# Pixel-Talk/CanonSwap

Measured on AMD Instinct MI355X. Metric: frames/sec at 512x512 (generator hot path F->W->T->R->W->G), higher is better.
Workload: dtype f16; 1 GPU; BASELINE configs[2]: 512x512 video, 64 frames batched per launch on each GPU, steady state over 1280 frames (20 launches per GPU) (256x256 crops in, random-init weights of the real architecture); frames_per_launch_per_gpu=64, frames_total=1280, parallelism=frame-shard x1, identities_resident=1, latency_mode=False, accumulate=fp32, debug_decodes=False

## Files before the change

canonswap_amd/_lib.py:

```python
from __future__ import annotations

import ctypes as C
import os
import subprocess

HERE = os.path.dirname(os.path.abspath(__file__))
CSRC = os.path.join(HERE, "csrc")
SOURCES = [os.path.join(CSRC, f) for f in ("conv_halo.hip", "conv_wide.hip", "conv_lat.hip", "vol32.hip", "vol32_fused.hip", "kernels.hip", "motion.hip", "imgops.hip", "engine.hip")]
TEST_SRC = os.path.join(os.path.dirname(HERE), "tests", "csrc", "test_igemm.hip")
TEST_LIB_PATH = os.path.join(os.path.dirname(HERE), "tests", "libcanonswap_test.so")
HEADERS = [os.path.join(CSRC, f) for f in ("common.h", "conv_epilogue.h", "conv_halo_kernel.h")] + \
          [os.path.join(os.path.dirname(HERE), "include", "canonswap_hip.h")]
HALO_NGROUPS = 8
OBJ_DIR = os.path.join(HERE, "build")
LIB_PATH = os.environ.get("CANONSWAP_LIB") or os.path.join(HERE, "libcanonswap_hip.so")
ABI_SYMBOLS = [
    "cs_create", "cs_destroy", "cs_last_error", "cs_abi_version", "cs_upload", "cs_finalize_weights", "cs_set_identity", "cs_set_latency_mode",
    "cs_extract_feature_3d", "cs_warp", "cs_warp_out", "cs_swap", "cs_swap_ids", "cs_swap_frames_ids", "cs_refine", "cs_warp_forward", "cs_spade_decode",
    "cs_pack_u8", "cs_unpack_u8", "cs_soft_erosion", "cs_prepare_crops", "cs_warp_affine_u8", "cs_warp_affine_f32", "cs_paste_back",
    "cs_motion_extract", "cs_motion_keypoints", "cs_soft_erosion_frames", "cs_paste_back_batch", "cs_swap_frames", "cs_animate_frames", 
    "cs_resize_half_bilinear", "cs_motion_keypoints_driven", "cs_paste_back_shared", "cs_crop_frames", "cs_face_masks", "cs_profile_begin", "cs_profile_end", "cs_profile_exec_flops", "cs_op_conv", "cs_op_grid_sample3d",
    "cs_op_chan_stats", "cs_op_chan_stats_partial_floats", "cs_op_pair_ragged", "cs_op_resblock3d", "cs_op_t_mask",
    "cs_op_t_style", "cs_op_t_modulate", "cs_op_t_read", "cs_op_t_layer",
    "cs_op_m_stem", "cs_op_m_dwln", "cs_op_m_ln_s2d", "cs_op_m_grn", "cs_op_m_head", "cs_op_m_pointwise",
# ... 105 lines not shown
            waits = waits[:4]
            loads = [(i, re.search(r"global_load_dwordx4 v\[(\d+):(\d+)\], v\[\d+:\d+\], off", l)) for i, l in enumerate(body)]
            loads = [(i, int(q.group(1))) for i, q in loads if q]
            prime = [r for i, r in loads if i < waits[0]][-4 * wch:]
            if len(prime) != 4 * wch:
                raise RuntimeError(f"isa_check: {name}: the prologue primes {len(prime)} ring registers, expected {4 * wch}")
            for k, w in enumerate(waits):
                slot = prime[k * wch:(k + 1) * wch]
                end = waits[k + 1] if k + 1 < 4 else len(body)
                seg = body[w:end]
                rel = [i for i, r in loads if w < i < end and r in slot]
                if len(rel) < wch:
                    raise RuntimeError(f"isa_check: {name}: ring slot {k} is not reloaded into v{slot} after its wait")
                first_reload = min(rel) - w
                uses = [j for j, l in enumerate(seg[:first_reload]) if "v_mfma" in l and any(f"v[{r}:{r + 3}]" in l for r in slot)]
                if not uses:
                    raise RuntimeError(f"isa_check: {name}: no MFMA reads ring slot {k} (v{slot}) between its wait and its reload")
            tail = "\n".join(body[waits[-1]:])
            if "s_waitcnt vmcnt(0)" not in tail:
                raise RuntimeError(f"isa_check: {name}: the ring is not drained (s_waitcnt vmcnt(0)) before the epilogue")
            seen[name] = len(waits)
    if not seen:
        raise RuntimeError("isa_check: no dynamic-shape conv_halo kernel found in the objects (name mangling changed?)")
    return seen


def _isa_check_lat(obj_dir: str, objdump: str) -> dict:
    import re
    oname = "conv_lat.o"
    obj = os.path.join(obj_dir, oname)
    subprocess.run([objdump, "--offloading", obj], check=True, capture_output=True)
    co = obj + ".0.hipv4-amdgcn-amd-amdhsa--gfx950"
    try:
        txt = subprocess.run([objdump, "-d", "--no-show-raw-insn", co], check=True, capture_output=True, text=True).stdout
    finally:
        for f in os.listdir(obj_dir):
            if f.startswith(oname + ".0."):
                os.remove(os.path.join(obj_dir, f))
    seen = {}
    for m in re.finditer(r"^[0-9a-f]+ <(\S*conv_lat_kernel\S*)>:\n(.*?)(?=^[0-9a-f]+ <|\Z)", txt, re.S | re.M):
        name, body = m.group(1), [l.split("//")[0].strip() for l in m.group(2).split("\n")]
        body = [l for l in body if l]
        mf = [i for i, l in enumerate(body) if l.startswith("v_mfma")]
        if not mf:
            raise RuntimeError(f"isa_check: {name}: no MFMA")
        if any(l.startswith(("s_cbranch", "s_branch")) for l in body[mf[0]:mf[-1]]):
            raise RuntimeError(f"isa_check: {name}: a branch inside the K loop (the walk assumes straight-line code)")
        for i, l in enumerate(body):
            if re.search(r"\bm0\b", l):
                ok = l.startswith("s_mov_b32 m0,") and any(b.startswith("buffer_load") and b.endswith("lds") for b in body[i + 1:i + 3])
                if not ok:
                    raise RuntimeError(f"isa_check: {name}: `{l}` touches m0 outside the hidden LDS-DMA sequence")
        nvm, open_dma, nbar, ndma = 0, [], 0, 0
        for i, l in enumerate(body[:mf[-1] + 1]):
            op = l.split()[0]
            if op.startswith(("global_load", "buffer_load", "global_store", "buffer_store", "scratch_load", "scratch_store")):
                if op.startswith("buffer_load") and l.endswith("lds"):
                    open_dma.append(nvm); ndma += 1
                nvm += 1
            if op == "s_barrier":
                nbar += 1
                w = next((body[j] for j in range(i - 1, max(i - 6, -1), -1) if body[j].startswith("s_waitcnt") and "vmcnt" in body[j]), None)
                if w is None and not open_dma:
                    continue
                if w is None:
                    raise RuntimeError(f"isa_check: {name}: barrier {nbar} of the K loop has no vmcnt wait in front of it")
                n = int(re.search(r"vmcnt\((\d+)\)", w).group(1))
                for idx in open_dma:
                    if nvm - idx - 1 < n:
                        raise RuntimeError(f"isa_check: {name}: `{w}` before barrier {nbar} does not cover a DMA piece issued {nvm - idx - 1} vector-memory instructions earlier")
                open_dma = []
        if open_dma:
            raise RuntimeError(f"isa_check: {name}: {len(open_dma)} DMA pieces are never waited for at a chunk head")
        if len(mf) not in (8 * 6 * 8, 8 * 6 * 16) or ndma != 24:
            raise RuntimeError(f"isa_check: {name}: {len(mf)} MFMAs / {ndma} DMA instructions, expected 384 or 768 / 24")
        seen[name] = len(mf)
    if not seen:
        raise RuntimeError("isa_check: no conv_lat kernel found in conv_lat.o (name mangling changed?)")
    return seen


def _isa_check_wide(obj_dir: str, objdump: str) -> dict:
    seen = _isa_check_ring(obj_dir, objdump, "conv_wide.o", r"\S*conv_wide_kernel\S*", 18 * 64)
    seen.update(_isa_check_ring(obj_dir, objdump, "conv_halo_g1.o", r"_Z16conv_halo_kernelILi32ELi8ELi5ELi2ELi2ELi0ELb1ELb0ELi[789]E\S*", None))
    return seen


def _isa_check_ring(obj_dir: str, objdump: str, oname: str, name_re: str, expect_mfma) -> dict:
    import re
    obj = os.path.join(obj_dir, oname)
    subprocess.run([objdump, "--offloading", obj], check=True, capture_output=True)
    co = obj + ".0.hipv4-amdgcn-amd-amdhsa--gfx950"
    try:
        txt = subprocess.run([objdump, "-d", "--no-show-raw-insn", co], check=True, capture_output=True, text=True).stdout
    finally:
        for f in os.listdir(obj_dir):
            if f.startswith(oname + ".0."):
                os.remove(os.path.join(obj_dir, f))
    seen = {}
    for m in re.finditer(r"^[0-9a-f]+ <(" + name_re + r")>:\n(.*?)(?=^[0-9a-f]+ <|\Z)", txt, re.S | re.M):
        name, body = m.group(1), m.group(2).split("\n")
        writer, waited, issued, nmfma = {}, {}, {}, 0
        pending, nvm = [], 0
        mf = [i for i, l in enumerate(body) if "v_mfma" in l]
        lo, hi = (mf[0], mf[-1]) if mf else (0, 0)
        for li, l in enumerate(body):
            t = l.split("//")[0].strip()
            if not t:
                continue
            op = t.split()[0]
            if op.startswith("s_waitcnt") and "vmcnt" in t:
                n = int(re.search(r"vmcnt\((\d+)\)", t).group(1))
                for r in waited:
                    if nvm - issued.get(r, -1) - 1 >= n:
                        waited[r] = True
                pending = [q for q in pending if nvm - q[1] - 1 < n]
            if op.startswith(("s_cbranch", "s_branch", "s_endpgm")) or li < lo:
                pending = []
            if pending and not op.startswith(("s_", "global_store", "buffer_store", "ds_write", "scratch_store")):
                mm0 = re.match(r"\S+\s+(v\[(\d+):(\d+)\]|v(\d+))", t)
                if mm0 and not (op.startswith("buffer_load") and t.endswith("lds")):
                    dst = set(range(int(mm0.group(2)), int(mm0.group(3)) + 1)) if mm0.group(2) else {int(mm0.group(4))}
                    for regs, _ in pending:
                        if regs & dst:
                            raise RuntimeError(f"isa_check: {name}: `{t}` writes v{sorted(regs & dst)} while an untracked ring load into them is in flight")
            if op.startswith(("global_load", "buffer_load", "global_store", "buffer_store", "scratch_load", "scratch_store", "global_atomic")):
                if op.startswith("global_load_dwordx4") and li >= lo:
                    q = re.match(r"\S+\s+v\[(\d+):(\d+)\]", t)
                    if q:
                        pending.append((set(range(int(q.group(1)), int(q.group(2)) + 1)), nvm))
                nvm += 1
            if op.startswith("v_mfma"):
                ops = re.findall(r"([av])\[(\d+):(\d+)\]", t)
                if len(ops) < 4 or ops[1][0] != "v":
                    raise RuntimeError(f"isa_check: {name}: MFMA with a weight operand outside the VGPRs: {t}")
                nmfma += 1
                for r in range(int(ops[1][1]), int(ops[1][2]) + 1):
                    if not writer.get(r, "").startswith("global_load_dwordx4"):
                        raise RuntimeError(f"isa_check: {name}: v{r}, a weight operand of `{t}`, was last written by `{writer.get(r)}` (a copy of a ring register?)")
                    if not waited.get(r, False):
                        raise RuntimeError(f"isa_check: {name}: no vmcnt wait between the ring load of v{r} and `{t}`")
                continue
            if op.startswith(("global_store", "buffer_store", "ds_write", "scratch_store", "s_", "buffer_load_dwordx4")) and "lds" in t + " lds" and not op.startswith("global_load"):
                if not op.startswith(("v_", "ds_read", "global_load", "scratch_load")):
                    continue
            mm = re.match(r"\S+\s+(v\[(\d+):(\d+)\]|v(\d+))", t)
            if mm and not op.startswith(("global_store", "buffer_store", "ds_write", "scratch_store")) and not (op.startswith("buffer_load") and t.endswith("lds")):
                rng = range(int(mm.group(2)), int(mm.group(3)) + 1) if mm.group(2) else [int(mm.group(4))]
                is_vm = op.startswith(("global_load", "buffer_load", "scratch_load"))
                for r in rng:
                    writer[r] = op
                    waited[r] = False
                    issued[r] = (nvm - 1) if is_vm else -1
        if expect_mfma is not None and nmfma != expect_mfma:
            raise RuntimeError(f"isa_check: {name}: {nmfma} MFMAs in the kernel, expected {expect_mfma}")
        seen[name] = nmfma
    if not seen:
        raise RuntimeError(f"isa_check: no kernel matching {name_re} found in {oname} (name mangling changed?)")
    return seen


class ConvDesc(C.Structure):
    _fields_ = [
        ("in_", C.c_void_p), ("in_sN", C.c_long), ("in_sD", C.c_long), ("in_sH", C.c_long), ("in_sW", C.c_long),
        ("N", C.c_int), ("D", C.c_int), ("H", C.c_int), ("W", C.c_int), ("Cin", C.c_int), ("up_shift", C.c_int),
        ("KD", C.c_int), ("KH", C.c_int), ("KW", C.c_int),
        ("wgt", C.c_void_p), ("Cout_pad", C.c_int), ("Cout", C.c_int),
# ... 106 lines not shown
```

canonswap_amd/csrc/common.h:

```cpp
#pragma once
#include <hip/hip_runtime.h>
#include <stdint.h>

typedef _Float16 half_t;
typedef _Float16 h8_t __attribute__((ext_vector_type(8)));
typedef _Float16 h4_t __attribute__((ext_vector_type(4)));
typedef float f4_t __attribute__((ext_vector_type(4)));

enum { ACT_NONE = 0, ACT_RELU = 1, ACT_LRELU = 2, ACT_SIGMOID = 3, ACT_GELU = 4 };
enum { MODE_STD = 0, MODE_TBLEND = 1, MODE_SPADE = 2, MODE_PIXSHUF = 3,
       MODE_STDSTAT = 4 };
enum { CFG_128x128 = 0, CFG_128x64 = 1, CFG_256x32 = 2, CFG_256x16 = 3 };
enum { CFG_H_128x128 = 10, CFG_H_128x64 = 11, CFG_H_256x32 = 12, CFG_H_128x32 = 13, CFG_H_128x16 = 14, CFG_H_256x16 = 15,
       CFG_H_SK128x32 = 16 , CFG_H_128x256 = 17,
       CFG_H_128x160 = 18 ,
       CFG_H_256x160 = 19 ,
       CFG_H_256x64 = 20 ,
       CFG_VOL32 = 30 , CFG_WIDE = 31 ,
       CFG_LAT = 32  };

struct TDesc {
    void* p;
    long sN, sD, sH, sW;
};

struct ConvParams {
    const half_t* in;
    const half_t* zero;
    long in_sN, in_sD, in_sH, in_sW;
    int N, D, H, W;
    int inD;
    int Cin;
    int cg, cg_cin;
    long in_sG;
    int nchunks;
    int up_shift;
    int KD, KH, KW, PD, PH, PW;
    const half_t* wgt;
    const long* wofs;
    const int* wslot;
    int Cout_pad;
    int Cout;
    int lgTW, lgTH, lgTD;
    int nTW, nTH, nTD, nTN;
    const float* bias;
    const float* bias2;
    int act0;
    float slope0;
    TDesc res;
    int res_f32;
    int res_shift;
    const float* pixscale;
    int ps_stride;
    TDesc out0;
    int out0_f32;
    const float* s2;
    const float* t2;
    int act1;
    float slope1;
    TDesc out1;
    const float* stats;
    float* stat_out;
    float* sk_out;
    int sk_splits;
    int ragged;
    unsigned mg_ncb, mg_tw, mg_th, mg_td;
    int hilo;
    int xcd_map;
    float* kw_out;
    int ep_general;
    int pool_hw;
    int spmul;
    const half_t* xs_w; TDesc xs_res, xs_out; int xs_cout;
    int persist_total;
    unsigned in_sample_bytes;
    int nphase;
    long ph_wofs[4];
    unsigned ph_ooff[4];
    int ph_PH[4], ph_PW[4];
    int xf_kind;
    int v32_srows;
    TDesc xf_y, xf_res, xf_out;
    const float* xf_stats; const float* xf_gamma; const float* xf_beta;
    float xf_slope;
#ifdef CS_TIMELINE
    unsigned long long* tl;
    long tl_cap;
#endif
};

__device__ __forceinline__ float gn_scale(float rstd, float gamma) { return rstd * gamma; }
__device__ __forceinline__ float gn_shift(float mean, float sc, float beta) { return fmaf(-mean, sc, beta); }
__device__ __forceinline__ float gn_lrelu(float v, float sc, float sh, float rr, float slope)
{
    float a = fmaf(v, sc, sh);
    a = a + rr;
    return fmaxf(a, a * slope);
}

#define CS_CHECK_HIP(expr)                                                                  \
// ... 87 lines not shown
```

canonswap_amd/csrc/conv_epilogue.h:

```cpp
#pragma once
#include "common.h"

#ifndef EP_TL
#define EP_TL(i) do { } while (0)
#endif
typedef unsigned int ep_u4_t __attribute__((ext_vector_type(4)));
typedef unsigned int ep_u2_t __attribute__((ext_vector_type(2)));

static inline int ep_check_extents(const ConvParams& p, const char* who)
{
    auto span = [&](const TDesc& t) -> long {
        return (long)(p.N - 1) * t.sN + (long)(p.D - 1) * t.sD + (long)(p.H - 1) * t.sH + (long)(p.W - 1) * t.sW + p.Cout;
    };
    auto wide = [&](const TDesc& t) { return t.sD >= (1L << 23) || t.sH >= (1L << 23) || t.sW >= (1L << 23); };
    const long lim = 1L << 31;
    long ph_max = 0;
    for (int z = 0; z < p.nphase && z < 4; ++z) ph_max = p.ph_ooff[z] > ph_max ? (long)p.ph_ooff[z] : ph_max;
    if ((p.out0.p && span(p.out0) + ph_max >= lim) || (p.out1.p && span(p.out1) >= lim) || (p.res.p && span(p.res) >= lim)) {
        cs_set_error("%s: a tensor of this launch spans 2^31 elements or more (32-bit in-tensor offsets)", who);
        return -1;
    }
    if ((p.out0.p && wide(p.out0)) || (p.out1.p && wide(p.out1)) || (p.res.p && wide(p.res)) || p.D >= (1 << 22) || p.H >= (1 << 22) ||
        p.W >= (1 << 22)) {
        cs_set_error("%s: an axis stride of 2^23 elements or more (24-bit multiplies in the addressing)", who);
// ... 97 lines not shown
#else
#define EP_STORE_COND
#endif
#define CONV_EPILOGUE_EARLY_FETCH() \
    ep_u2_t ep_xpre[EP_EARLY ? EP_WPX0 : 1][EP_EARLY ? (WCH + 1) / 2 : 1]; \
    if constexpr (EP_EARLY) { \
        int xlw, xlh, xld, xln; \
        { int t = l15p; xlw = t & mW; t >>= lgTW; xlh = t & mH; t >>= lgTH; xld = t & mD; t >>= lgTD; xln = t; } \
        const int xrs = p.res_shift, xnb = tn * (BM >> lgS); \
        const unsigned xlane = (unsigned)((xnb + xln) * (int)p.res.sN + __mul24((td << lgTD) + xld, (int)p.res.sD) + \
                                          __mul24(((th << lgTH) + xlh) >> xrs, (int)p.res.sH) + __mul24(((tw << lgTW) + xlw) >> xrs, (int)p.res.sW)); \
_Pragma("unroll") \
        for (int pi = 0; pi < EP_WPX0; ++pi) { \
            int bw, bh, bd, bn; \
            { int t = (ep_wpx0 * EP_WPX0 + pi) << 4; bw = t & mW; t >>= lgTW; bh = t & mH; t >>= lgTH; bd = t & mD; t >>= lgTD; bn = t; } \
            const unsigned xb = xlane + (unsigned)(bn * (int)p.res.sN + bd * (int)p.res.sD + (bh >> xrs) * (int)p.res.sH + (bw >> xrs) * (int)p.res.sW); \
_Pragma("unroll") \
            for (int ci = 0; ci < WCH; ci += 2) { \
                const int cb = ep_chan(EP_PAIR, 2, n0 + wch * WCH * 16, ci, l4); \
                ep_u2_t q2; q2[0] = 0u; q2[1] = 0u; \
                if (p.res.p && xnb + xln + bn < p.N && cb < p.Cout) q2 = *(const ep_u2_t*)((const half_t*)p.res.p + (xb + (unsigned)cb)); \
                ep_xpre[pi][ci / 2] = q2; \
            } \
        } \
    }

template <int N> __device__ __forceinline__ float ep_row_shl(float a)
{
#ifdef EP_HOST_EMULATION
    (void)a;
    return 0.f;
#else
    return __builtin_bit_cast(float, __builtin_amdgcn_update_dpp(0, __builtin_bit_cast(int, a), 0x100 | N, 0xf, 0xf, true));
#endif
}

__device__ __forceinline__ float ep_row_sum16(float a)
{
#ifdef EP_HOST_EMULATION
    for (int o = 1; o < 16; o <<= 1) a += __shfl_xor(a, o, 64);
    return a;
#else
    a += __builtin_bit_cast(float, __builtin_amdgcn_update_dpp(0, __builtin_bit_cast(int, a), 0x101, 0xf, 0xf, true));
    a += __builtin_bit_cast(float, __builtin_amdgcn_update_dpp(0, __builtin_bit_cast(int, a), 0x102, 0xf, 0xf, true));
    a += __builtin_bit_cast(float, __builtin_amdgcn_update_dpp(0, __builtin_bit_cast(int, a), 0x104, 0xf, 0xf, true));
    a += __builtin_bit_cast(float, __builtin_amdgcn_update_dpp(0, __builtin_bit_cast(int, a), 0x108, 0xf, 0xf, true));
    return a;
#endif
}

#define EP_STAT_FLUSH(sg) \
    if (EP_STAT) { \
        const int ep_tiles = p.nTW * p.nTH * p.nTD; \
        const int ep_nblk = EP_NBLK_V; \
        const int ep_blk = EP_BLK_V(sg); \
_Pragma("unroll") \
        for (int ci = 0; ci < WCH; ci += CSTEP) { \
            const int cb = ep_chan(EP_PAIR, CSTEP, n0 + wch * WCH * 16, ci, l4); \
            float ep_pa[4], ep_pb[4]; \
_Pragma("unroll") \
            for (int r = 0; r < 4; ++r) { \
                ep_pa[r] = ep_row_sum16(ep_sum[EP_STAT ? ci : 0][r]); ep_pb[r] = ep_row_sum16(ep_sq[EP_STAT ? ci : 0][r]); \
                ep_sum[EP_STAT ? ci : 0][r] = 0.f; ep_sq[EP_STAT ? ci : 0][r] = 0.f; \
            } \
             \
            if (l15 == 0 && cb < p.Cout) { \
                float4* dst = (float4*)(p.stat_out + (((long)tn * ep_nblk + ep_blk) * p.Cout + cb) * 2); \
                dst[0] = make_float4(ep_pa[0], ep_pb[0], ep_pa[1], ep_pb[1]); \
                dst[1] = make_float4(ep_pa[2], ep_pb[2], ep_pa[3], ep_pb[3]); \
            } \
        } \
    }

#ifndef EP_GSEL_V
#define EP_GSEL_V 0
#endif
#ifndef EP_BLK_V
#define EP_BLK_V(sg) ((tile_lin % ep_tiles) * (BM / (EP_SG * 16)) + ep_wpx * (EP_WPX / EP_SG) + (sg))
#define EP_NBLK_V (ep_tiles * (BM / (EP_SG * 16)))
#endif
#ifndef EP_SLICE_FENCE
#define EP_SLICE_FENCE
#endif
#ifndef EP_FG
#define EP_FG 8
#endif
#ifndef EP_FG_F32
#define EP_FG_F32 4
#endif
#ifndef EP_FG_STAT
#define EP_FG_STAT 4
#endif
#ifndef EP_PIPE_V
#define EP_PIPE_V 0
#endif
#ifndef EP_O0_EXTRA_V
#define EP_O0_EXTRA_V 0u
#endif
#ifndef EP_POOL_WSH_V
#define EP_POOL_WSH_V 0
#define EP_POOL_HSH_V 0
#endif
#define EP_POOLB 128
#ifndef EP_SPMUL_V
#define EP_SPMUL_V 0
#endif
#ifndef EP_O1ONLY_V
#define EP_O1ONLY_V 0
#endif
#ifndef EP_MLIN_V
#define EP_MLIN_V 0
#endif
#ifndef EP_DUP_V
#define EP_DUP_V 0
#endif
#define EP_SPMULB 256
#define EP_GELUB 512
#define EP_FETCH_ROUND(PG0, BI) \
    if (EP_PF && !EP_EARLY && (ep_fetch || ep_has_ps)) { \
_Pragma("unroll") \
        for (int g = 0; g < EP_G; ++g) { \
            int bw, bh, bd, bn; \
            { int t = (ep_wpx * EP_WPX + (PG0) + g) << 4; bw = t & mW; t >>= lgTW; bh = t & mH; t >>= lgTH; bd = t & mD; t >>= lgTD; bn = t; } \
            if (!EPFAST && ep_nb + ep_ln + bn >= p.N) continue; \
            if (ep_has_ps) ep_ps2[BI][g] = p.pixscale[ep_lane_ps + (unsigned)((((bn * p.D + bd) * p.H + bh) * p.W + bw) * p.ps_stride)]; \
            if (ep_fetch) { \
                const unsigned xb = ep_lane_res + (unsigned)(bn * (int)p.res.sN + bd * (int)p.res.sD + (bh >> ep_rs) * (int)p.res.sH + \
                                                            (bw >> ep_rs) * (int)p.res.sW); \
_Pragma("unroll") \
                for (int ci = 0; ci < WCH; ci += CSTEP) { \
                    const int cb = ep_chan(EP_PAIR, CSTEP, n0 + wch * WCH * 16, ci, l4); \
                    if (!EPALL && cb >= p.Cout) continue; \
                    if (ep_res32) ep_raw2[BI][g][(EP_PF ? ci / CSTEP : 0)] = *(const ep_u4_t*)((const float*)p.res.p + (xb + (unsigned)cb)); \
                    else if (ep_mr && ep_second(EP_PAIR, ci)) {  } \
                    else if (ep_mr && (EPALL || cb + 4 < p.Cout)) ep_raw2[BI][g][(EP_PF ? ci / CSTEP : 0)] = *(const ep_u4_t*)((const half_t*)p.res.p + (xb + (unsigned)cb)); \
                    else { \
                        const ep_u2_t q2 = *(const ep_u2_t*)((const half_t*)p.res.p + (xb + (unsigned)cb)); \
                        ep_raw2[BI][g][(EP_PF ? ci / CSTEP : 0)][0] = q2[0]; ep_raw2[BI][g][(EP_PF ? ci / CSTEP : 0)][1] = q2[1]; \
                    } \
                } \
            } \
        } \
    }
#define CONV_EPILOGUE_IMPL(EPCODE) \
    constexpr int EPF = (EPCODE); \
    constexpr bool EPFAST = EPF >= 0; \
    constexpr bool EPALL = EPFAST && ((EPF >> 6) & 1) == 0;       \
    constexpr bool EP_POOL = EPFAST && ((EPF >> 7) & 1) != 0 && (EP_POOL_WSH_V) > 0;       \
    constexpr int EP_PS = EP_POOL ? 1 : 0; \
    constexpr bool EP_GELU = EPFAST && ((EPF >> 9) & 1) != 0;           \
    const bool ep_spm = EPFAST ? (((EPF >> 8) & 1) != 0) : ((MODE == MODE_STD) && p.spmul != 0); \
    constexpr bool EP_POOL_HB = EP_POOL && (EP_POOL_HSH_V) == 0;       \
    float ep_phold[EP_POOL_HB ? WCH : 1][4];                            \
    const bool ep_has_res = EPFAST ? ((EPF & 3) != 0) : (p.res.p != nullptr); \
    const bool ep_res32 = EPFAST ? ((EPF & 3) == 2) : (p.res_f32 != 0); \
    const bool ep_has_o0 = EPFAST ? (((EPF >> 2) & 1) != 0) : (p.out0.p != nullptr); \
    const bool ep_o032 = EPFAST ? (((EPF >> 3) & 1) != 0) : (p.out0_f32 != 0); \
    const bool ep_has_o1 = EPFAST ? (((EPF >> 4) & 1) != 0) : (p.out1.p != nullptr); \
    const bool ep_has_ps = EPFAST ? (((EPF >> 5) & 1) != 0) : (p.pixscale != nullptr); \
    constexpr int CSTEP = (MODE == MODE_TBLEND || MODE == MODE_SPADE) ? 2 : 1; \
     \
    float4 ep_bias[WCH], ep_bias2[WCH], ep_s2[WCH], ep_t2[WCH], ep_mean[WCH], ep_rstd[WCH]; \
_Pragma("unroll") \
    for (int ci = 0; ci < WCH; ci += CSTEP) { \
        const int cb = ep_chan(EP_PAIR, CSTEP, n0 + wch * WCH * 16, ci, l4); \
        const bool cok = EPALL || cb < p.Cout; \
        ep_bias[ci] = (cok && p.bias) ? *(const float4*)(p.bias + cb) : make_float4(0.f, 0.f, 0.f, 0.f); \
        ep_bias2[ci] = (cok && MODE == MODE_SPADE) ? *(const float4*)(p.bias2 + cb) : make_float4(0.f, 0.f, 0.f, 0.f); \
        ep_s2[ci] = (cok && p.s2) ? *(const float4*)(p.s2 + cb) : make_float4(1.f, 1.f, 1.f, 1.f); \
        ep_t2[ci] = (cok && p.s2) ? *(const float4*)(p.t2 + cb) : make_float4(0.f, 0.f, 0.f, 0.f); \
        if ((MODE == MODE_SPADE || ep_spm) && cok) {  \
            const float4 q0 = *(const float4*)(p.stats + ((long)tn * p.Cout + cb) * 2); \
            const float4 q1 = *(const float4*)(p.stats + ((long)tn * p.Cout + cb) * 2 + 4); \
            ep_mean[ci] = make_float4(q0.x, q0.z, q1.x, q1.z); ep_rstd[ci] = make_float4(q0.y, q0.w, q1.y, q1.w); \
        } else { ep_mean[ci] = make_float4(0.f, 0.f, 0.f, 0.f); ep_rstd[ci] = make_float4(1.f, 1.f, 1.f, 1.f); } \
    } \
    const float ep_sl0 = lin_slope(p.act0, p.slope0), ep_sl1 = lin_slope(p.act1, p.slope1); \
    constexpr bool EP_STAT = (MODE == MODE_STDSTAT);  \
    constexpr int EP_SC = EP_STAT ? WCH : 1; \
     \
    constexpr int EP_SG = EP_WPX > 4 ? 4 : EP_WPX; \
    float ep_sum[EP_SC][4], ep_sq[EP_SC][4]; \
_Pragma("unroll") \
    for (int ci = 0; ci < EP_SC; ++ci) \
_Pragma("unroll") \
        for (int r = 0; r < 4; ++r) { ep_sum[ci][r] = 0.f; ep_sq[ci][r] = 0.f; } \
     \
    constexpr bool EP_PF = (WCH != 5); \
     \
    constexpr int EP_G = (EP_GSEL_V) > 0 ? (EP_GSEL_V) : !EP_PF ? 1 : (EP_WPX < 8 ? EP_WPX : (MODE == MODE_TBLEND ? 8 : (WCH == 4 ? (EPFAST ? (EP_STAT ? EP_FG_STAT : ((EPF & 3) == 2 ? EP_FG_F32 : EP_FG)) : (EP_STAT ? 1 : 2)) : 4))); \
    constexpr int EP_NCI = EP_PF ? (WCH + CSTEP - 1) / CSTEP : 1; \
    const bool ep_fetch = EP_PF && ep_has_res; \
     \
    const bool ep_m0 = EP_PAIR != 0 && !ep_o032 && (EPFAST || ep_al8(p.out0)); \
    const bool ep_m1 = EP_PAIR != 0 && (EPFAST || ep_al8(p.out1)); \
    const bool ep_mr = EP_PAIR != 0 && EP_PF && !ep_res32 && (EPFAST || ep_al8(p.res)); \
    const int ep_rshift = (MODE == MODE_SPADE || ep_spm) ? p.res_shift : 0; \
     \
    int ep_lw, ep_lh, ep_ld, ep_ln; \
    { int t = l15p; ep_lw = t & mW; t >>= lgTW; ep_lh = t & mH; t >>= lgTH; ep_ld = t & mD; t >>= lgTD; ep_ln = t; } \
    const int ep_w0 = tw << lgTW, ep_h0 = th << lgTH, ep_d0 = td << lgTD, ep_nb = tn * (BM >> lgS); \
    const int ep_rs = (MODE == MODE_SPADE || ep_spm) ? p.res_shift : 0; \
     \
    const bool ep_tn1 = (BM >> lgS) == 1; \
    const unsigned ep_lane_res = (unsigned)(ep_nb * (int)p.res.sN + (ep_tn1 ? 0 : ep_ln * (int)p.res.sN) + __mul24(ep_d0 + ep_ld, (int)p.res.sD) + \
                                            __mul24((ep_h0 + ep_lh) >> ep_rs, (int)p.res.sH) + __mul24((ep_w0 + ep_lw) >> ep_rs, (int)p.res.sW)); \
    const unsigned ep_lane_o0 = (EP_O0_EXTRA_V) + (unsigned)(ep_nb * (int)p.out0.sN + (ep_tn1 ? 0 : ep_ln * (int)p.out0.sN) + __mul24(ep_d0 + ep_ld, (int)p.out0.sD) + \
                                           __mul24((ep_h0 + ep_lh) >> EP_PS, (int)p.out0.sH) + __mul24((ep_w0 + ep_lw) >> EP_PS, (int)p.out0.sW)); \
     \
    const bool ep_pool_lane = !EP_POOL || (lane & ((EP_POOL_WSH_V) | (EP_POOL_HSH_V))) == 0; \
    const unsigned ep_lane_o1 = (EP_O0_EXTRA_V) + (unsigned)(ep_nb * (int)p.out1.sN + (ep_tn1 ? 0 : ep_ln * (int)p.out1.sN) + __mul24(ep_d0 + ep_ld, (int)p.out1.sD) + \
                                           __mul24(ep_h0 + ep_lh, (int)p.out1.sH) + __mul24(ep_w0 + ep_lw, (int)p.out1.sW)); \
    const unsigned ep_lane_ps = (unsigned)(((((ep_nb + ep_ln) * p.D + ep_d0 + ep_ld) * p.H + ep_h0 + ep_lh) * p.W + ep_w0 + ep_lw) * p.ps_stride); \
     \
    const unsigned ep_lane_px = (unsigned)((((ep_nb + ep_ln) * 3) * 2 * p.H + 2 * (ep_h0 + ep_lh)) * 2 * p.W + 2 * (ep_w0 + ep_lw)); \
     \
    constexpr bool EP_PIPE = (EP_PIPE_V) != 0 && EP_G < EP_WPX; \
    ep_u4_t ep_raw2[EP_PIPE ? 2 : 1][EP_G][EP_NCI]; float ep_ps2[EP_PIPE ? 2 : 1][EP_G]; \
    if (EP_PIPE) { EP_FETCH_ROUND(0, 0) } \
_Pragma("unroll") \
    for (int pg = 0; pg < EP_WPX; pg += EP_G) { \
    const int ep_bi = EP_PIPE ? ((pg / EP_G) & 1) : 0; \
    if (!EP_PIPE) { EP_FETCH_ROUND(pg, 0) } \
    else if (pg + EP_G < EP_WPX) { EP_FETCH_ROUND(pg + EP_G, EP_PIPE ? (((pg / EP_G) + 1) & 1) : 0) } \
    ep_u4_t (&ep_raw)[EP_G][EP_NCI] = ep_raw2[ep_bi]; float (&ep_ps)[EP_G] = ep_ps2[ep_bi]; \
    if (pg == 0) EP_TL(6); \
_Pragma("unroll") \
    for (int g = 0; g < EP_G; ++g) { \
        const int pi = pg + g; \
        if (pi == 1) EP_TL(7); \
        if (pi > 0 && pi % EP_SG == 0) { EP_STAT_FLUSH(pi / EP_SG - 1) } \
        int bw, bh, bd, bn; \
        { int t = (ep_wpx * EP_WPX + pi) << 4; bw = t & mW; t >>= lgTW; bh = t & mH; t >>= lgTH; bd = t & mD; t >>= lgTD; bn = t; } \
        if (!EPFAST && ep_nb + ep_ln + bn >= p.N) continue; \
        float ps = 1.f; \
        if (ep_has_ps) ps = EP_PF ? ep_ps[g] : p.pixscale[ep_lane_ps + (unsigned)((((bn * p.D + bd) * p.H + bh) * p.W + bw) * p.ps_stride)]; \
        const unsigned xb = ep_lane_res + (unsigned)(bn * (int)p.res.sN + bd * (int)p.res.sD + (bh >> ep_rs) * (int)p.res.sH + (bw >> ep_rs) * (int)p.res.sW); \
        const unsigned ob0 = ep_lane_o0 + (unsigned)(bn * (int)p.out0.sN + bd * (int)p.out0.sD + (bh >> EP_PS) * (int)p.out0.sH + (bw >> EP_PS) * (int)p.out0.sW); \
        const unsigned ob1 = ep_lane_o1 + (unsigned)(bn * (int)p.out1.sN + bd * (int)p.out1.sD + bh * (int)p.out1.sH + bw * (int)p.out1.sW); \
        float ep_vh[4] = {0.f, 0.f, 0.f, 0.f}, ep_uh[4] = {0.f, 0.f, 0.f, 0.f};       \
_Pragma("unroll") \
        for (int ci = 0; ci < WCH; ci += CSTEP) { \
            const int cb = ep_chan(EP_PAIR, CSTEP, n0 + wch * WCH * 16, ci, l4); \
            if (!EPALL && cb >= p.Cout) continue; \
            float rr[4] = {0.f, 0.f, 0.f, 0.f};      \
            if (ep_has_res) { \
                if (EP_EARLY) { \
                    const h4_t hx = __builtin_bit_cast(h4_t, ep_xpre[EP_EARLY ? pi : 0][EP_EARLY ? ci / 2 : 0]); \
_Pragma("unroll") \
                    for (int r = 0; r < 4; ++r) rr[r] = (float)hx[r]; \
                } else if (EP_PF) { \
                    const bool ep_hi = ep_mr && ep_second(EP_PAIR, ci);       \
                    const ep_u4_t q4 = ep_raw[g][(EP_PF ? ci / CSTEP : 0)]; \
                    const ep_u4_t qp = ep_raw[g][(EP_PF && ep_second(EP_PAIR, ci) ? ci / CSTEP - 1 : 0)]; \
                    if (ep_res32) { \
                        const f4_t qf = __builtin_bit_cast(f4_t, q4);      \
_Pragma("unroll") \
                        for (int r = 0; r < 4; ++r) rr[r] = qf[r]; \
                    } else { \
                        ep_u2_t q2; q2[0] = ep_hi ? qp[2] : q4[0]; q2[1] = ep_hi ? qp[3] : q4[1]; \
                        const h4_t hx = __builtin_bit_cast(h4_t, q2); \
_Pragma("unroll") \
                        for (int r = 0; r < 4; ++r) rr[r] = (float)hx[r]; \
                    } \
                } else { \
                    load4(p.res, ep_res32, (long)(xb + (unsigned)cb), rr); \
                } \
            } \
            float v[4]; \
            if (MODE == MODE_TBLEND) { \
_Pragma("unroll") \
                for (int r = 0; r < 4; ++r) \
                    v[r] = ps * (ep_acc[ci + CSTEP - 1][pi][r] + ((const float*)&ep_bias[ci])[r]) + (1.f - ps) * ep_acc[ci][pi][r]; \
            } else if (MODE == MODE_SPADE) { \
_Pragma("unroll") \
                for (int r = 0; r < 4; ++r) { \
                    const float gm = ep_acc[ci][pi][r] + ((const float*)&ep_bias[ci])[r]; \
                    const float bt = ep_acc[ci + CSTEP - 1][pi][r] + ((const float*)&ep_bias2[ci])[r]; \
                    v[r] = fmaf((rr[r] - ((const float*)&ep_mean[ci])[r]) * ((const float*)&ep_rstd[ci])[r], 1.f + gm, bt); \
                } \
            } else { \
_Pragma("unroll") \
                for (int r = 0; r < 4; ++r) v[r] = ep_acc[ci][pi][r] + ((const float*)&ep_bias[ci])[r]; \
                if (ep_spm) { \
_Pragma("unroll") \
                    for (int r = 0; r < 4; ++r) v[r] = ((rr[r] - ((const float*)&ep_mean[ci])[r]) * ((const float*)&ep_rstd[ci])[r]) * (1.f + v[r]); \
                } \
            } \
_Pragma("unroll") \
             \
            for (int r = 0; r < 4; ++r) v[r] = EP_GELU ? gelu_act(v[r]) : ((EP_HEAVY && !EPFAST) ? apply_act(v[r], p.act0, p.slope0) : lin_act(v[r], ep_sl0)); \
            if (MODE == MODE_PIXSHUF) { \
                const int c = cb >> 2; \
                if (c < 3) { \
                    float* o = (float*)p.out0.p; \
                    const unsigned W2 = 2u * (unsigned)p.W, H2 = 2u * (unsigned)p.H; \
                    const unsigned base = ep_lane_px + ((unsigned)(bn * 3 + c) * H2 + 2u * (unsigned)bh) * W2 + 2u * (unsigned)bw; \
                    *(float2*)(o + base) = make_float2(v[0], v[1]); \
                    *(float2*)(o + base + W2) = make_float2(v[2], v[3]); \
                } \
                continue; \
            } \
             \
            if (MODE != MODE_SPADE && !ep_spm) { \
_Pragma("unroll") \
                for (int r = 0; r < 4; ++r) v[r] += rr[r]; \
            } \
            if (MODE == MODE_STD || MODE == MODE_STDSTAT) { \
_Pragma("unroll") \
                for (int r = 0; r < 4; ++r) v[r] *= ps; \
            } \
            if (EP_POOL_HB) {  \
_Pragma("unroll") \
                for (int r = 0; r < 4; ++r) { \
                    if ((pi & 1) == 0) ep_phold[EP_POOL_HB ? ci : 0][r] = v[r]; \
                    else { \
// ... 105 lines not shown
```

canonswap_amd/csrc/conv_halo.hip:

```cpp
#include "conv_halo_kernel.h"

#ifndef HALO_GROUP
#define HALO_GROUP (-1)
#endif
#define IN_GROUP(g) (HALO_GROUP == -1 || HALO_GROUP == (g))
#define NOT_MINE (-2)

template <int CK, int WPX, int WCH, int WVP, int WVC, int MODE, bool SK, int STV>
static int launch_halo_cfg(const ConvParams& p, hipStream_t st)
{
    if constexpr (STV != 0) {
        using SS = StaticShape<STV>;
        if (p.KD == SS::KD && p.KH == SS::KH && p.KW == SS::KW && p.lgTW == SS::LW && p.lgTH == SS::LH && p.lgTD == SS::LD &&
            p.nchunks % (CK / 32) == 0)
            return launch_halo_st<CK, WPX, WCH, WVP, WVC, MODE, SK, STV>(p, st);
    }
    if constexpr (WCH == 4 && MODE == MODE_STDSTAT) {
        cs_set_error("conv_halo: the 128x256 statistics tile exists for the static shapes only (%dx%dx%d taps, tile 2^%d x 2^%d x 2^%d)",
                     p.KD, p.KH, p.KW, p.lgTW, p.lgTH, p.lgTD);
        return -1;
    } else {
        return launch_halo_st<CK, WPX, WCH, WVP, WVC, MODE, SK, 0>(p, st);
    }
}

#define HALO_CASE(CFG, WPX, WCH, WVP, WVC, MODE, SK, ST2D, ST3D)                                         \
    if (cfg == CFG && mode == MODE) {                                                                    \
        if (ck == 64) return launch_halo_cfg<64, WPX, WCH, WVP, WVC, MODE, SK, ST2D>(p, st);            \
        if (stv == 1) return launch_halo_cfg<32, WPX, WCH, WVP, WVC, MODE, SK, ST2D>(p, st);            \
        if (stv == 5 && ST3D == 2) return launch_halo_cfg<32, WPX, WCH, WVP, WVC, MODE, SK, (ST3D == 2 ? 5 : 0)>(p, st); \
        return launch_halo_cfg<32, WPX, WCH, WVP, WVC, MODE, SK, ST3D>(p, st);                           \
    }

#define GROUP_FN(g) int launch_conv_halo_g##g(const ConvParams& p, int cfg, int ck, int mode, int stv, hipStream_t st)
GROUP_FN(0); GROUP_FN(1); GROUP_FN(2); GROUP_FN(3); GROUP_FN(4); GROUP_FN(5); GROUP_FN(6); GROUP_FN(7);

#if IN_GROUP(0)
GROUP_FN(0)
{
    (void)stv;
    if (p.KD == 3 && p.KH == 2 && p.KW == 2 && ck == 32 && mode == MODE_STD) {
        if (cfg == CFG_H_256x32) return launch_halo_cfg<32, 4, 2, 4, 1, MODE_STD, false, 12>(p, st);
        if (cfg == CFG_H_128x64) return launch_halo_cfg<32, 4, 2, 2, 2, MODE_STD, false, 13>(p, st);
        if (cfg == CFG_H_128x128 && p.lgTW == 2) return launch_halo_cfg<32, 8, 2, 1, 4, MODE_STD, false, 17>(p, st);
        if (cfg == CFG_H_128x128) return launch_halo_cfg<32, 8, 2, 1, 4, MODE_STD, false, 13>(p, st);
    }
    if (mode == MODE_STD && p.KD == 1 && p.KH == 1 && p.KW == 1) {
        if (cfg == CFG_H_128x128 && ck == 32) return launch_halo_cfg<32, 8, 2, 1, 4, MODE_STD, false, 15>(p, st);
        if (cfg == CFG_H_128x64 && ck == 64) return launch_halo_cfg<64, 4, 2, 2, 2, MODE_STD, false, 15>(p, st);
        if (cfg == CFG_H_128x64 && ck == 32) return launch_halo_cfg<32, 4, 2, 2, 2, MODE_STD, false, 15>(p, st);
        if (cfg == CFG_H_128x32 && ck == 64) return launch_halo_cfg<64, 2, 2, 4, 1, MODE_STD, false, 15>(p, st);
        if (cfg == CFG_H_128x32 && ck == 32) return launch_halo_cfg<32, 2, 2, 4, 1, MODE_STD, false, 15>(p, st);
    }
    return NOT_MINE;
}
#endif

#if IN_GROUP(1)
GROUP_FN(1)
{
    if (cfg == CFG_H_128x128 && mode == MODE_STD && ck == 64 && p.KD == 1 && p.KH <= 2 && p.KW <= 2) {
        if (p.KH == 2 && p.KW == 2) return launch_halo_cfg<64, 8, 2, 1, 4, MODE_STD, false, 10>(p, st);
        if (p.KH == 2) return launch_halo_cfg<64, 8, 2, 1, 4, MODE_STD, false, 11>(p, st);
        if (p.KW == 2) return launch_halo_cfg<64, 8, 2, 1, 4, MODE_STD, false, 14>(p, st);
        return launch_halo_cfg<64, 8, 2, 1, 4, MODE_STD, false, 15>(p, st);
    }
    if (cfg == CFG_H_256x64 && mode == MODE_STD && ck == 32) return launch_halo_cfg<32, 8, 2, 2, 2, MODE_STD, false, 7>(p, st);
    if (cfg == CFG_H_256x64 && ck == 64) {
        if (p.KD != 1 || p.KH != 3 || p.KW != 3 || p.lgTW != 4 || p.lgTH != 4 || p.lgTD != 0) {
            cs_set_error("conv_halo: the 2-D 256x64 tile runs 3x3 convs on 16x16 tiles only");
            return -1;
        }
        if (mode == MODE_STD) return launch_halo_st<64, 8, 2, 2, 2, MODE_STD, false, 16>(p, st);
        if (mode == MODE_STDSTAT) return launch_halo_st<64, 8, 2, 2, 2, MODE_STDSTAT, false, 16>(p, st);
    }
    if (cfg == CFG_H_256x160 && mode == MODE_STD && ck == 32) {
        if (p.KD == 7 && p.lgTW == 2) return launch_halo_cfg<32, 8, 5, 2, 2, MODE_STD, false, 9>(p, st);
        if (p.KD == 7) return launch_halo_cfg<32, 8, 5, 2, 2, MODE_STD, false, 8>(p, st);
        return launch_halo_cfg<32, 8, 5, 2, 2, MODE_STD, false, 7>(p, st);
    }
    if (cfg == CFG_H_128x160 && mode == MODE_STD && ck == 32) {
        if (stv == 4) return launch_halo_cfg<32, 4, 5, 2, 2, MODE_STD, false, 4>(p, st);
        if (stv == 6) return launch_halo_cfg<32, 4, 5, 2, 2, MODE_STD, false, 6>(p, st);
        return launch_halo_cfg<32, 4, 5, 2, 2, MODE_STD, false, 2>(p, st);
    }
    return NOT_MINE;
}
#endif

#if IN_GROUP(2)
GROUP_FN(2)
{
    HALO_CASE(CFG_H_128x256, 8, 4, 1, 4, MODE_STD, false, 1, 0)
    HALO_CASE(CFG_H_128x256, 8, 4, 1, 4, MODE_TBLEND, false, 1, 0)
    return NOT_MINE;
}
#endif

#if IN_GROUP(3)
GROUP_FN(3)
{
    HALO_CASE(CFG_H_128x256, 8, 4, 1, 4, MODE_SPADE, false, 1, 0)
    HALO_CASE(CFG_H_128x256, 8, 4, 1, 4, MODE_STDSTAT, false, 1, 0)
    return NOT_MINE;
}
#endif

#if IN_GROUP(4)
GROUP_FN(4)
{
    HALO_CASE(CFG_H_128x128, 8, 2, 1, 4, MODE_STD, false, 1, 2)
    HALO_CASE(CFG_H_128x128, 8, 2, 1, 4, MODE_STDSTAT, false, 1, 0)
    return NOT_MINE;
}
#endif

#if IN_GROUP(5)
GROUP_FN(5)
{
    HALO_CASE(CFG_H_128x128, 8, 2, 1, 4, MODE_TBLEND, false, 1, 0)
    HALO_CASE(CFG_H_128x128, 8, 2, 1, 4, MODE_SPADE, false, 1, 0)
    HALO_CASE(CFG_H_128x64, 4, 2, 2, 2, MODE_STDSTAT, false, 1, 0)
    return NOT_MINE;
}
#endif

#if IN_GROUP(6)
GROUP_FN(6)
{
    HALO_CASE(CFG_H_128x64, 4, 2, 2, 2, MODE_STD, false, 1, 2)
    HALO_CASE(CFG_H_256x32, 4, 2, 4, 1, MODE_STD, false, 0, 3)
    HALO_CASE(CFG_H_256x32, 4, 2, 4, 1, MODE_STDSTAT, false, 0, 3)
    return NOT_MINE;
}
#endif

#if IN_GROUP(7)
GROUP_FN(7)
{
    HALO_CASE(CFG_H_128x32, 2, 2, 4, 1, MODE_STD, false, 0, 2)
    HALO_CASE(CFG_H_128x16, 2, 1, 4, 1, MODE_STD, false, 1, 0)
    HALO_CASE(CFG_H_256x16, 4, 1, 4, 1, MODE_PIXSHUF, false, 0, 0)
    HALO_CASE(CFG_H_SK128x32, 8, 2, 4, 1, MODE_STD, true, 0, 0)
    return NOT_MINE;
}
#endif

#if IN_GROUP(0) && defined(CS_TIMELINE)
unsigned long long* g_cs_tl = nullptr;
long g_cs_tl_cap = 0;
extern "C" void cs_debug_set_timeline(void* buf, long cap) { g_cs_tl = (unsigned long long*)buf; g_cs_tl_cap = cap; }
#endif

#if IN_GROUP(0)
int launch_conv_halo(const ConvParams& p, int cfg, int ck, int mode, hipStream_t st)
{
    if (mode == MODE_STD && p.stat_out) mode = MODE_STDSTAT;
    const int stv = p.KD == 1 ? 1 : (p.KD == 7 ? (p.lgTW == 1 ? 6 : 4) : (p.lgTD == 4 ? 3 : (p.lgTD == 3 ? 5 : 2)));
    int r;
#define TRY_GROUP(g) if ((r = launch_conv_halo_g##g(p, cfg, ck, mode, stv, st)) != NOT_MINE) return r;
    TRY_GROUP(0) TRY_GROUP(1) TRY_GROUP(2) TRY_GROUP(3) TRY_GROUP(4) TRY_GROUP(5) TRY_GROUP(6) TRY_GROUP(7)
#undef TRY_GROUP
// ... 5 lines not shown
```

canonswap_amd/csrc/conv_halo_kernel.h:

```cpp
#pragma once
#include <type_traits>
#include <utility>
#include <cstdlib>
#include "common.h"
#ifdef CS_TIMELINE
#define EP_TL(i) TL_STAMP(i)
#endif
#define EP_POOL_WSH_V EP_POOL_WSH_K
#define EP_POOL_HSH_V EP_POOL_HSH_K
#define EP_SPMUL_V EP_SPMUL_K
#define EP_DUP_V EP_DUP_K
#define EP_MLIN_V EP_MLIN_K
#define EP_O1ONLY_V EP_O1ONLY_K
#define EP_O0_EXTRA_V ep_o0_extra
#include "conv_epilogue.h"

typedef unsigned int u4_t __attribute__((ext_vector_type(4)));
__device__ __forceinline__ unsigned mdiv(unsigned u, unsigned magic) { return magic ? __umulhi(u, magic) : u; }

template <int OFF>
__device__ __forceinline__ void wfrag_load(u4_t& dst, const half_t* ptr)
{
    asm volatile("global_load_dwordx4 %0, %1, off offset:%2" : "=v"(dst) : "v"(ptr), "n"(OFF));
}
template <int N>
__device__ __forceinline__ void wait_vmcnt_le()
{
    asm volatile("s_waitcnt vmcnt(%0)" ::"n"(N) : "memory");
}

#ifdef CS_TIMELINE
extern unsigned long long* g_cs_tl;
extern long g_cs_tl_cap;
#define TL_STAMP(i) do { __builtin_amdgcn_sched_barrier(0); tl_t[i] = __builtin_amdgcn_s_memtime(); __builtin_amdgcn_sched_barrier(0); } while (0)
#else
#define TL_STAMP(i) do { } while (0)
#endif

template <int ST> struct StaticShape { static constexpr int KD = 0, KH = 0, KW = 0, LW = 0, LH = 0, LD = 0; };
template <> struct StaticShape<1> { static constexpr int KD = 1, KH = 3, KW = 3, LW = 4, LH = 3, LD = 0; };
template <> struct StaticShape<2> { static constexpr int KD = 3, KH = 3, KW = 3, LW = 3, LH = 3, LD = 1; };
template <> struct StaticShape<3> { static constexpr int KD = 3, KH = 3, KW = 3, LW = 2, LH = 2, LD = 4; };
template <> struct StaticShape<4> { static constexpr int KD = 7, KH = 7, KW = 1, LW = 3, LH = 3, LD = 1; };
template <> struct StaticShape<5> { static constexpr int KD = 3, KH = 3, KW = 3, LW = 2, LH = 2, LD = 3; };
template <> struct StaticShape<6> { static constexpr int KD = 7, KH = 7, KW = 1, LW = 1, LH = 3, LD = 3; };
template <> struct StaticShape<7> { static constexpr int KD = 3, KH = 3, KW = 3, LW = 3, LH = 3, LD = 2; };
template <> struct StaticShape<8> { static constexpr int KD = 7, KH = 7, KW = 1, LW = 1, LH = 3, LD = 4; };
template <> struct StaticShape<9> { static constexpr int KD = 7, KH = 7, KW = 1, LW = 2, LH = 3, LD = 3; };
template <> struct StaticShape<16> { static constexpr int KD = 1, KH = 3, KW = 3, LW = 4, LH = 4, LD = 0; };
template <> struct StaticShape<12> { static constexpr int KD = 3, KH = 2, KW = 2, LW = 2, LH = 2, LD = 4; };
template <> struct StaticShape<13> { static constexpr int KD = 3, KH = 2, KW = 2, LW = 3, LH = 3, LD = 1; };
template <> struct StaticShape<17> { static constexpr int KD = 3, KH = 2, KW = 2, LW = 2, LH = 2, LD = 3; };
template <> struct StaticShape<10> { static constexpr int KD = 1, KH = 2, KW = 2, LW = 4, LH = 3, LD = 0; };
template <> struct StaticShape<11> { static constexpr int KD = 1, KH = 2, KW = 1, LW = 4, LH = 3, LD = 0; };
template <> struct StaticShape<14> { static constexpr int KD = 1, KH = 1, KW = 2, LW = 4, LH = 3, LD = 0; };
template <> struct StaticShape<15> { static constexpr int KD = 1, KH = 1, KW = 1, LW = 4, LH = 3, LD = 0; };

template <int CK, int WPX, int WCH, int WVP, int ST, int MODE> constexpr int halo_pad()
{
#ifdef CS_LDS_V1
    return 1;
#else
    if (CK == 64 && WCH == 4 && WPX == 8 && ST == 1) return 2;
    if (CK == 32 && WCH == 5 && WPX == 8 && (ST == 7 || ST == 8 || ST == 9)) return 2;
    if (CK == 64 && WCH == 2 && WPX == 8 && WVP == 2 && ST == 16) return 2;
    if (CK == 32 && WCH == 2 && WPX == 8 && ST == 1 && MODE == MODE_SPADE) return 2;
#ifdef CS_LDS_V32
    if (CK == 32 && WCH == 2 && WPX == 4 && WVP == 4 && ST == 3) return 2;
#endif
    return 1;
#endif
}
template <int ST, int PAD> constexpr int halo_hi()
{
    if (PAD == 2) return ST == 3 ? 16 : (ST == 9 ? 19 : ((ST == 7 || ST == 8) ? 15 : (ST == 16 ? 13 : 8)));
    return ST == 4 ? 18 : ((ST == 3 || ST == 7 || ST == 8 || ST == 9) ? 13 : (ST == 12 ? 9 : 8));
}
template <int ST, int PAD> __host__ __device__ constexpr int halo_lane_pos(int l)
{
#ifdef CS_LDS_V1
    return l;
#else
    using SS = StaticShape<ST>;
    if (ST == 0 || SS::KW != 3 || SS::LW > 3 || SS::LW < 2) return l;
    if (SS::LW == 2 && PAD == 2) return ((l & 1) << 1) | ((l & 2) << 2) | ((l >> 2) & 1) | ((l & 8) >> 1);
    return ((l & 1) << 1) | ((l & 2) << 1) | ((l >> 2) & 1) | (l & 8);
#endif
}

template <class F, int... I> __device__ __forceinline__ void halo_static_for_impl(F&& f, std::integer_sequence<int, I...>) { (f(std::integral_constant<int, I>{}), ...); }
template <int N, class F> __device__ __forceinline__ void halo_static_for(F&& f) { halo_static_for_impl(static_cast<F&&>(f), std::make_integer_sequence<int, N>{}); }

template <int WCH, int PFS, int HI, int ST0>
constexpr int halo_ring_young(int st, int L, int NP, bool dma_cur)
{
    auto dma = [&](int u, bool on) { return (on && u >= ST0 && u < ST0 + HI) ? 1 : 0; };
    auto cur_before = [&](int from_step ) {
        int n = 0;
        for (int u = from_step; u < st; ++u) n += (u >= 1 ? WCH : 0) + dma(u, dma_cur);
        return n;
    };
    if (st >= PFS) {
        const int u0 = st - PFS + 1;
        return dma(u0, dma_cur) + cur_before(u0 + 1);
    }
    const int prime = (PFS - 1 - st) * WCH + cur_before(0);
    int g = 0;
    if (NP % PFS == 0) g = st + NP - PFS + 1;
    else { for (int u = NP - PFS + 1; u <= NP; ++u) if ((u - 1) % PFS == st) g = u; }
    int carried = dma(g, true);
    for (int u = g + 1; u <= NP; ++u) carried += WCH + (u < NP ? dma(u, true) : 0);
    carried += cur_before(0);
    return prime < carried ? prime : carried;
}

template <int ST, int PAD> constexpr int halo_pool_shift(int bit)
{
    for (int b = 0; b < 4; ++b) if (halo_lane_pos<ST, PAD>(1 << b) == (1 << bit)) return 1 << b;
    return 0;
}

template <int WCH, int ST> constexpr bool halo_phase_group() { return !(ST == 0 && WCH >= 4); }

template <int CK, int WPX, int WCH, int WVP, int MODE, bool SK, int ST> constexpr bool halo_pool2d()
{
    using SS = StaticShape<ST>;
    return ST != 0 && !SK && MODE == MODE_STD && CK == 32 && WPX == 8 && WVP == 1 && (WCH == 2 || WCH == 4) && SS::KD == 1 && SS::KH == 3 && SS::KW == 3 &&
           SS::LW == 4 && SS::LH == 3 && SS::LD == 0;
}

template <int CK, int WPX, int WCH, int WVP, int WVC, int MODE, bool DB, bool SK, int ST>
__global__ void __launch_bounds__(256, (WCH == 4 ? 2 : ((WCH == 2 && WPX == 8 && !SK && ST != 0) ? (WVP == 2 ? 2 : 3) : 1))) conv_halo_kernel(const ConvParams p)
{
    using SS = StaticShape<ST>;
    static_assert(ST == 0 || !SK, "static shapes are not combined with split-K");
    constexpr int BM = SK ? WPX * 16 : WPX * 16 * WVP;
    constexpr int BN = WCH * 16 * WVC;
    constexpr int SL = CK / 8;
    constexpr int PAD = halo_pad<CK, WPX, WCH, WVP, ST, MODE>();
    constexpr int SLP = SL + PAD;
    constexpr bool EP_POOLK = ST != 0 && !SK && MODE == MODE_STD && WCH == 2 && SS::KD == 3 && SS::KH == 3 && SS::KW == 3 && (SS::LW == 3 || SS::LW == 2) && SS::LH >= 1;
    constexpr bool EP_POOLK2 = halo_pool2d<CK, WPX, WCH, WVP, MODE, SK, ST>();
    constexpr bool XSK = ST == 1 && !SK && MODE == MODE_STD && CK == 64 && WCH == 4 && WPX == 8 && WVP == 1;
#ifdef CS_NO_SPMUL_FAST
    constexpr bool EP_SPMUL_K = false;
#else
    constexpr bool EP_SPMUL_K = ST == 1 && !SK && MODE == MODE_STD && CK == 64 && WCH == 4 && WPX == 8 && WVP == 1;
#endif
    constexpr bool EP_O1ONLY_K = ST == 16 && !SK && MODE == MODE_STD;
    constexpr bool EP_MLIN_K = ST == 15 && !SK && MODE == MODE_STD;
    constexpr bool EP_DUP_K = (ST == 11 || ST == 14 || ST == 15) && !SK && MODE == MODE_STD && WCH == 2 && WPX == 8;
    constexpr int EP_POOL_WSH_K = EP_POOLK ? halo_pool_shift<ST, PAD>(0) : (EP_POOLK2 ? 1 : 0);
    constexpr int EP_POOL_HSH_K = EP_POOLK ? halo_pool_shift<ST, PAD>(SS::LW) : 0;
    constexpr int VS = SLP * 16;
    constexpr int HI = halo_hi<ST, PAD>();
    constexpr int KH32 = CK / 32;
    constexpr int PFD = 4;
    constexpr int SKS = SK ? 4 : 1;
    static_assert(WVP * WVC == 4, "4 waves per workgroup");
    static_assert(!SK || (WVC == 1 && WPX == 8), "split-K variants: every wave covers all 128 positions");

    extern __shared__ __attribute__((aligned(16))) unsigned char smem[];
#ifdef CS_TIMELINE
    unsigned long long tl_t[8] = {0, 0, 0, 0, 0, 0, 0, 0};
    const unsigned long long tl_real0 = __builtin_amdgcn_s_memrealtime();
    TL_STAMP(0);
#endif

#ifdef CS_DEPHASE
    if (MODE == MODE_SPADE && WCH == 4) {
        unsigned hwid;
        asm volatile("s_getreg_b32 %0, hwreg(HW_REG_HW_ID)" : "=s"(hwid));
        if ((hwid & 1u) && (int)(blockIdx.x + blockIdx.y * gridDim.x) < 512)
            for (int i = 0; i < CS_DEPHASE; ++i) __builtin_amdgcn_s_sleep(16);
    }
#endif
    const int tid = threadIdx.x, lane = tid & 63;
    const int wave = __builtin_amdgcn_readfirstlane(tid >> 6);
    constexpr bool PHK = halo_phase_group<WCH, ST>();
    const int phz = (PHK && p.nphase) ? (int)blockIdx.z : 0;
    const int PHv = (PHK && p.nphase) ? p.ph_PH[phz] : p.PH, PWv = (PHK && p.nphase) ? p.ph_PW[phz] : p.PW;
    const unsigned ep_o0_extra = (PHK && p.nphase) ? p.ph_ooff[phz] : 0u;
    const int wpx = SK ? 0 : wave % WVP, wch = SK ? 0 : wave / WVP;
    const int l15 = lane & 15, l4 = lane >> 4;
    const int l15p = halo_lane_pos<ST, PAD>(l15);
#ifdef CS_NO_PAIR
    constexpr int EP_PAIR = 0;
#else
    constexpr int EP_PAIR = ep_pair_of(MODE, WCH);
#endif

#ifdef CS_NO_ASMRING
    constexpr bool ASMRK = false;
#else
    constexpr bool ASMRK = DB && !SK && CK == 32 && WCH == 5 && WPX == 8 && WVP == 2 && (ST == 7 || ST == 8 || ST == 9) && MODE == MODE_STD;
#endif
    u4_t wr_p[ASMRK ? 3 : 1][ASMRK ? WCH : 1];
    unsigned poffb[ASMRK ? HI : 1];
    __amdgpu_buffer_rsrc_t rsrc_p;
    int gbuf = 0;
    bool staged = false;
    const bool persist = ASMRK && p.persist_total > 0;
    int p_base = 0, p_cnt = 0, p_j = 0, p_i = 0, p_per = 1;
    if (persist) {
        const int total = p.persist_total, G = (int)gridDim.x;
        const int xcd = blockIdx.x & 7, q = total >> 3, r = total & 7;
        p_i = blockIdx.x >> 3; p_per = G >> 3;
        p_base = xcd * q + (xcd < r ? xcd : r); p_cnt = q + (xcd < r ? 1 : 0);
        if (p_i >= p_cnt) return;
    }
    for (;;) {
    int tile_lin = blockIdx.x, cblk = blockIdx.y;
    const bool has_next = persist && p_i + p_per * (p_j + 1) < p_cnt;
    auto u_to_tile = [&](int u, int& tl_, int& cb_) {
        const int ncb = p.Cout_pad / BN;
        tl_ = (int)mdiv((unsigned)u, p.mg_ncb); cb_ = u - tl_ * ncb;
    };
    if (persist) u_to_tile(p_base + p_i + p_per * p_j, tile_lin, cblk);
    else if (p.xcd_map != 0) {
        const int flat = p.xcd_map == 2;
        const int total = (int)gridDim.x;
        const int xcd = blockIdx.x & 7, i = blockIdx.x >> 3;
        const int q = total >> 3, r = total & 7;
        const int u = xcd * q + (xcd < r ? xcd : r) + i;
        if (flat) u_to_tile(u, tile_lin, cblk);
        else tile_lin = u;
    }
    int t = tile_lin, tq;
    tq = (int)mdiv((unsigned)t, p.mg_tw); const int tw = t - tq * p.nTW; t = tq;
    tq = (int)mdiv((unsigned)t, p.mg_th); const int th = t - tq * p.nTH; t = tq;
    tq = (int)mdiv((unsigned)t, p.mg_td); const int td = t - tq * p.nTD; t = tq;
    const int tn = t;
    const int n0 = cblk * BN;
    const int lgTW = ST ? SS::LW : p.lgTW, lgTH = ST ? SS::LH : p.lgTH, lgTD = ST ? SS::LD : p.lgTD;
    const int KD = ST ? SS::KD : p.KD, KH = ST ? SS::KH : p.KH, KW = ST ? SS::KW : p.KW;
    const int lgS = lgTW + lgTH + lgTD;
    const int mW = (1 << lgTW) - 1, mH = (1 << lgTH) - 1, mD = (1 << lgTD) - 1;
    const int TN = BM >> lgS;
    const int HW = (1 << lgTW) + KW - 1, HH = (1 << lgTH) + KH - 1, HD = (1 << lgTD) + KD - 1;
    const int HV = TN * HD * HH * HW;
    const int nitems = HV * SLP;
    const int w0 = tw << lgTW, h0 = th << lgTH, d0 = td << lgTD, nb = tn * TN;
    const int ntaps = KD * KH * KW;

    const int isN = (int)p.in_sN, isD = (int)p.in_sD, isH = (int)p.in_sH, isW = (int)p.in_sW;
    const int in_nb = nb * isN;
    auto piece_off = [&](int q, bool& inb) -> int {
        const int hv = q / SLP;
        const int hw = hv % HW; int r = hv / HW;
        const int hh = r % HH; r /= HH;
        const int hd = r % HD;
        const int hn = TN == 1 ? 0 : r / HD;
        const int n = nb + hn, id = d0 + hd - p.PD, ih = h0 + hh - PHv, iw = w0 + hw - PWv;
        inb = q < nitems && (q % SLP) < SL && (TN == 1 ? r < HD : true) && n < p.N && (unsigned)id < (unsigned)p.D &&
              (unsigned)ih < (unsigned)p.H && (unsigned)iw < (unsigned)p.W;
        return in_nb + (TN == 1 ? 0 : hn * isN) + __mul24(id, isD) + __mul24(ih >> p.up_shift, isH) + __mul24(iw >> p.up_shift, isW) +
               (q % SLP) * 8;
    };
    const bool pre = DB || nitems <= 256 * HI;
    int poff[HI];
    unsigned pmask = 0;
    if (pre) {
#pragma unroll
        for (int j = 0; j < HI; ++j) {
            bool inb;
            const int o = piece_off(tid + 256 * j, inb);
            poff[j] = inb ? o : 0;
            pmask |= inb ? (1u << j) : 0u;
        }
    }
    auto glds = [&](const half_t* src, int buf, int q_wave_base) {
        __builtin_amdgcn_global_load_lds((const __attribute__((address_space(1))) void*)src,
                                         (__attribute__((address_space(3))) void*)(smem + (size_t)buf * HV * VS + (size_t)q_wave_base * 16),
                                         16, 0, 0);
    };
    auto stage_halo = [&](int buf, int c0) {
        long coff = c0;
        int climit = p.Cin - c0;
        if ((CK == 32 || ST == 15 || (ST == 0 && WCH != 4)) && p.cg > 0) {
            const int j = c0 >> 5;
            coff = (long)(j / p.cg) * p.in_sG + (j % p.cg) * 32;
            climit = p.cg_cin - (j % p.cg) * 32;
        }
        if (pre) {
#pragma unroll
            for (int j = 0; j < HI; ++j) {
                const int q = tid + 256 * j;
                if (q < nitems) {
                    const bool ok = ((pmask >> j) & 1u) && ((q % SLP) * 8 < climit);
                    glds(ok ? p.in + poff[j] + coff : p.zero, buf, 256 * j + wave * 64);
                }
            }
        } else if constexpr (!DB) {
            for (int q0 = 0; q0 < nitems; q0 += 256) {
                const int q = q0 + tid;
                if (q < nitems) {
                    bool inb;
                    const int o = piece_off(q, inb);
                    const bool ok = inb && ((q % SLP) * 8 < climit);
                    glds(ok ? p.in + o + coff : p.zero, buf, q0 + wave * 64);
                }
            }
        }
    };

    int abase[WPX];
#pragma unroll
    for (int pi = 0; pi < WPX; ++pi) {
        int m = wpx * WPX * 16 + pi * 16 + l15p;
        const int wl = m & mW; m >>= lgTW;
        const int hl = m & mH; m >>= lgTH;
        const int dl = m & mD; m >>= lgTD;
        abase[pi] = (((m * HD + dl) * HH + hl) * HW + wl) * VS + l4 * 16;
    }
    const int nck = (p.Cin + CK - 1) / CK;
    const int j0 = SK ? wave : 0;
    int cc_lo = 0, cc_hi = nck;
    if (p.sk_out) { cc_lo = (int)(((long)nck * blockIdx.z) / gridDim.z); cc_hi = (int)(((long)nck * (blockIdx.z + 1)) / gridDim.z); }

    const half_t* wbase = p.wgt;
    if (p.wslot) wbase += p.wofs[p.wslot[nb < p.N ? nb : p.N - 1]];
    if (PHK && p.nphase) wbase += p.ph_wofs[phz];
    const half_t* wlane = wbase + ((long)(n0 + wch * WCH * 16) * 32 + ep_lane_row(EP_PAIR, l15) * 32 + l4 * 8);
    const long wstep = (long)p.Cout_pad * 32;

#ifdef CS_NO_EARLY
    constexpr bool EP_EARLY = false;
#else
    constexpr bool EP_EARLY = (MODE == MODE_SPADE) && !SK && ST != 0 && WCH == 2 && WPX == 8;
#endif
#ifdef CS_NO_EPFAST
    constexpr bool EP_FAST = false;
#else
    constexpr bool EP_FAST = !SK && ST != 0 && (WCH == 4 || WCH == 5 || (WCH == 2 && WPX == 8) || ST == 15);
#endif
    constexpr int EP_WPX0 = WPX;
    const int ep_wpx0 = wpx;
    CONV_EPILOGUE_EARLY_FETCH()

    f4_t acc[WCH][WPX];
#pragma unroll
    for (int ci = 0; ci < WCH; ++ci)
#pragma unroll
        for (int pi = 0; pi < WPX; ++pi) acc[ci][pi] = (f4_t){0.f, 0.f, 0.f, 0.f};

    if constexpr (ST != 0) {
        constexpr int NT = SS::KD * SS::KH * SS::KW, NS = NT * KH32;
        constexpr bool RAGK = (CK == 32) && (WPX == 8) && (ST == 7 || ST == 8 || ST == 9) && MODE == MODE_STD;
        constexpr bool LATK = CK == 64 && WCH == 2 && WPX == 4 && ST == 1 && !SK;
#ifdef CS_PFS3
        constexpr int PFS = NS < 3 ? NS : 3;
#else
        constexpr int PFS = NS < 3 ? NS : (WCH * WPX <= 4 ? (NS < 8 ? NS : 8) : (LATK ? (NS < 6 ? NS : 6) : 3));
#endif
#ifdef CS_NO_WCARRY
        constexpr bool WCARRY = false;
#else
#ifdef CS_WCARRY_MULT
        constexpr bool WCARRY = (NS % PFS == 0) && NS >= 2 * PFS && WPX == 8 && WVP == 2;
#else
        constexpr bool WCARRY = NS >= 2 * PFS && ((WPX == 8 && WVP == 2) || LATK);
#endif
#endif
        constexpr int SHW = (1 << SS::LW) + SS::KW - 1, SHH = (1 << SS::LH) + SS::KH - 1;
#ifdef CS_NO_ASMRING
        constexpr bool ASMR = false;
#else
        constexpr bool ASMR = DB && WCH == 5 && WPX == 8 && WVP == 2 && (ST == 7 || ST == 8 || ST == 9) && MODE == MODE_STD && PFS == 3;
#endif
        if constexpr (ASMR) {
            static_assert(SK == false && KH32 == 1, "ASMR: 32-channel chunks");
            constexpr int HSTRIDE = HI * 4096;
            constexpr int ST0 = 1;
            constexpr unsigned OOB = 0x80000000u;
            static_assert(ASMRK, "the kernel-level and the block-level conditions of ASMR agree");
            auto (&wr) = wr_p;
            auto set_stage = [&](int n_, int d0_, int h0_, int w0_) {
                rsrc_p = __builtin_amdgcn_make_buffer_rsrc((void*)(p.in + (long)n_ * p.in_sN), 0, (int)p.in_sample_bytes, 0x00020000);
                int tid_o = tid;
                asm volatile("" : "+v"(tid_o));
#pragma unroll
                for (int j = 0; j < HI; ++j) {
                    const int q = tid_o + 256 * j;
                    const int hv = q / SLP, sl = q % SLP;
                    const int hw = hv % HW; int r = hv / HW;
                    const int hh = r % HH; r /= HH;
                    const int id = d0_ + r - p.PD, ih = h0_ + hh - PHv, iw = w0_ + hw - PWv;
                    const bool inb = q < nitems && sl < SL && r < HD && (unsigned)id < (unsigned)p.D && (unsigned)ih < (unsigned)p.H && (unsigned)iw < (unsigned)p.W;
                    poffb[j] = inb ? (unsigned)(__mul24(id, isD) + __mul24(ih >> p.up_shift, isH) + __mul24(iw >> p.up_shift, isW) + sl * 8) * 2u : OOB;
                }
            };
            auto stage_piece = [&](int buf, int cn, int j) {
                const bool nxt = cn >= cc_hi;
                const int c0 = (nxt ? cc_lo : cn) * CK;
                const int climit = (nxt && !has_next) ? 0 : p.Cin - c0;
                const unsigned off = (((tid + 256 * j) % SLP) * 8 < climit) ? poffb[j] : OOB;
                __builtin_amdgcn_raw_ptr_buffer_load_lds(rsrc_p, (__attribute__((address_space(3))) void*)(smem + (size_t)buf * HSTRIDE + (size_t)(256 * j + wave * 64) * 16),
                                                         16, (int)off, c0 * 2, 0, 0);
            };
            auto wsrc_of = [&](int cc, int st, int nsc) -> const half_t* {
                int c2 = cc, s2 = st;
                if (st >= nsc) { c2 = cc + 1; s2 = (nsc % PFS == 0) ? st - nsc : (st - PFS) % PFS; }
                const int ccl = c2 < cc_hi ? c2 : cc_lo;
                return wlane + (long)(ccl * NT + s2) * wstep;
            };
            auto wload1 = [&](u4_t& dst, const half_t* src, int ci) {
                if (ci == 0) asm volatile("global_load_dwordx4 %0, %1, off" : "=v"(dst) : "v"(src));
                else if (ci == 1) asm volatile("global_load_dwordx4 %0, %1, off offset:1024" : "=v"(dst) : "v"(src));
                else if (ci == 2) asm volatile("global_load_dwordx4 %0, %1, off offset:2048" : "=v"(dst) : "v"(src));
                else if (ci == 3) asm volatile("global_load_dwordx4 %0, %1, off offset:3072" : "=v"(dst) : "v"(src));
                else asm volatile("global_load_dwordx4 %0, %1, off" : "=v"(dst) : "v"(src + 4 * 16 * 32));
            };
            static_assert(EP_PAIR == 0, "ASMR: plain weight row order");
            TL_STAMP(1);
            constexpr bool CARRY = ST != 9;
            if (!staged) {
                set_stage(nb, d0, h0, w0);
#pragma unroll
                for (int j = 0; j < HI; ++j) stage_piece(gbuf, cc_lo, j);
            }
            if (!staged || !CARRY) {
#pragma unroll
                for (int st = 0; st < PFS; ++st)
#pragma unroll
                    for (int ci = 0; ci < WCH; ++ci) wload1(wr[st][ci], wsrc_of(cc_lo, st, NS), ci);
            }
            TL_STAMP(2);
            auto run_chunk_a = [&](int cc, auto rag_t) {
                constexpr bool RAG = decltype(rag_t)::value;
                wait_vmcnt_le<PFS * WCH>();
                __builtin_amdgcn_s_barrier();
                asm volatile("" ::: "memory");
                const unsigned char* hb = smem + (size_t)gbuf * HSTRIDE;
                const int nbuf = gbuf ^ 1;
                gbuf ^= 1;
                if (cc + 1 == cc_hi && has_next) {
                    int ntl, ncb_, t2 = 0, q2;
                    u_to_tile(p_base + p_i + p_per * (p_j + 1), ntl, ncb_);
                    t2 = ntl;
                    q2 = (int)mdiv((unsigned)t2, p.mg_tw); const int tw2 = t2 - q2 * p.nTW; t2 = q2;
                    q2 = (int)mdiv((unsigned)t2, p.mg_th); const int th2 = t2 - q2 * p.nTH; t2 = q2;
                    q2 = (int)mdiv((unsigned)t2, p.mg_td); const int td2 = t2 - q2 * p.nTD; t2 = q2;
                    set_stage(t2 * TN, td2 << lgTD, th2 << lgTH, tw2 << lgTW);
                }
                constexpr int HA = WPX / 2;
                constexpr int PK = SS::KW > 1 ? SS::KW : SS::KH, SPR = PK / 2 + PK % 2;
                constexpr int NSC = RAG ? (NT / PK) * SPR : NS;
                auto tap_of = [&](int st) -> int { return RAG ? (st / SPR) * PK + 2 * (st % SPR) : st; };
                auto paired = [&](int st) -> bool { return RAG && (st % SPR) < PK / 2; };
                auto toff_of = [&](int st) -> int {
                    const int tap = tap_of(st);
                    return (((tap / (SS::KW * SS::KH)) * SHH + (tap / SS::KW) % SS::KH) * SHW + tap % SS::KW) * VS;
                };
                int abP[RAG ? WPX : 1];
                if constexpr (RAG) {
                    const int pd = (l4 >= 2) ? (SS::KW > 1 ? VS : SHW * VS) - 32 : 0;
#pragma unroll
                    for (int pi = 0; pi < WPX; ++pi) abP[pi] = abase[pi] + pd;
                }
                auto ab_of = [&](int pi, int st) -> int { return paired(st) ? abP[RAG ? pi : 0] : abase[pi]; };
                h8_t afA[HA], afB[WPX - HA];
#pragma unroll
                for (int pi = 0; pi < HA; ++pi) afA[pi] = *(const h8_t*)(hb + ab_of(pi, 0) + toff_of(0));
                halo_static_for<NSC>([&](auto stc) {
                    constexpr int st = decltype(stc)::value;
                    {
#ifdef CS_ASMR_DEBUG0
                        constexpr int NY = 0;
#else
                        constexpr int NY = halo_ring_young<WCH, PFS, HI, ST0>(st, NSC, NS, true);
#endif
                        asm volatile("s_waitcnt vmcnt(%5)" : "+v"(wr[st % PFS][0]), "+v"(wr[st % PFS][1]), "+v"(wr[st % PFS][2]), "+v"(wr[st % PFS][3]),
                                                             "+v"(wr[st % PFS][4]) : "n"(NY));
                    }
                    __builtin_amdgcn_sched_barrier(0);
                    const half_t* rsrc_w = wsrc_of(cc, st - 1 + PFS, NSC);
                    const int toff = toff_of(st);
#pragma unroll
                    for (int k = 0; k < 2 * WCH; ++k) {
                        const int ci = k >> 1, p0 = (k & 1) * 2;
                        acc[ci][p0] = __builtin_amdgcn_mfma_f32_16x16x32_f16(__builtin_bit_cast(h8_t, wr[st % PFS][ci]), afA[p0], acc[ci][p0], 0, 0, 0);
                        acc[ci][p0 + 1] = __builtin_amdgcn_mfma_f32_16x16x32_f16(__builtin_bit_cast(h8_t, wr[st % PFS][ci]), afA[p0 + 1], acc[ci][p0 + 1], 0, 0, 0);
                        if (k >= 2 && k < 6) afB[k - 2] = *(const h8_t*)(hb + ab_of(HA + k - 2, st) + toff);
                        if constexpr (st >= 1) { if (k >= 5) wload1(wr[(st - 1) % PFS][k - 5], rsrc_w, k - 5); }
                        __builtin_amdgcn_sched_barrier(0);
                    }
                    if (st >= ST0 && st < ST0 + HI) { stage_piece(nbuf, cc + 1, st - ST0); __builtin_amdgcn_sched_barrier(0); }
#pragma unroll
                    for (int k = 0; k < 2 * WCH; ++k) {
                        const int ci = k >> 1, p0 = (k & 1) * 2;
                        acc[ci][HA + p0] = __builtin_amdgcn_mfma_f32_16x16x32_f16(__builtin_bit_cast(h8_t, wr[st % PFS][ci]), afB[p0], acc[ci][HA + p0], 0, 0, 0);
                        acc[ci][HA + p0 + 1] = __builtin_amdgcn_mfma_f32_16x16x32_f16(__builtin_bit_cast(h8_t, wr[st % PFS][ci]), afB[p0 + 1], acc[ci][HA + p0 + 1], 0, 0, 0);
                        if (k >= 2 && k < 6 && st + 1 < NSC) afA[k - 2] = *(const h8_t*)(hb + ab_of(k - 2, st + 1) + toff_of(st + 1));
                        __builtin_amdgcn_sched_barrier(0);
                    }
                });
                {
                    const half_t* rsrc_w = wsrc_of(cc, NSC - 1 + PFS, NSC);
#pragma unroll
                    for (int ci = 0; ci < WCH; ++ci) wload1(wr[(NSC - 1) % PFS][ci], rsrc_w, ci);
                }
            };
            const bool rag = RAGK && p.ragged && cc_hi == nck;
            for (int cc = cc_lo; cc < cc_hi - (rag ? 1 : 0); ++cc) run_chunk_a(cc, std::false_type{});
            if constexpr (RAGK) {
                if (rag) run_chunk_a(cc_hi - 1, std::true_type{});
            }
            staged = has_next;
            if (!has_next || !CARRY) {
                wait_vmcnt_le<0>();
                __builtin_amdgcn_sched_barrier(0);
            }
#pragma unroll
            for (int st = 0; st < PFS; ++st)
                asm volatile("" :: "v"(wr[st][0]), "v"(wr[st][1]), "v"(wr[st][2]), "v"(wr[st][3]), "v"(wr[st][4]));
        } else {
        u4_t wr[PFS][WCH];
        auto wload_at = [&](u4_t (&dst)[WCH], int cc, int st) {
            const int ccl = cc < nck ? cc : nck - 1;
            const half_t* src = wlane + (long)((ccl * KH32 + st % KH32) * NT + st / KH32) * wstep;
#pragma unroll
            for (int ci = 0; ci < WCH; ++ci) dst[ci] = *(const u4_t*)(src + ep_frag_row(EP_PAIR, ci) * 32);
        };
        TL_STAMP(1);
        stage_halo(0, cc_lo * CK);
        __syncthreads();
        TL_STAMP(2);
        if (DB && cc_lo + 1 < cc_hi) stage_halo(1, (cc_lo + 1) * CK);
        auto chunk_head = [&](int cc) -> const unsigned char* {
            if (!WCARRY || cc == cc_lo) {
#pragma unroll
                for (int st = 0; st < PFS; ++st) wload_at(wr[st], cc, st);
            }
            if (cc > cc_lo && !(p.hilo && cc == 1)) {
                if (DB) {
                    __syncthreads();
                    if (cc + 1 < cc_hi) stage_halo((cc + 1 - cc_lo) & 1, (cc + 1) * CK);
                } else {
                    __syncthreads();
                    stage_halo(0, (p.hilo ? 1 : cc) * CK);
                    __syncthreads();
                }
            }
            return smem + (size_t)(DB ? ((cc - cc_lo) & 1) : 0) * HV * VS;
        };
        auto run_chunk = [&](int cc, const unsigned char* hb, auto rag_t) {
            constexpr bool RAG = decltype(rag_t)::value;
            constexpr int HA = WPX / 2;
            constexpr int PK = SS::KW > 1 ? SS::KW : SS::KH, SPR = PK / 2 + PK % 2;
            constexpr int NSC = RAG ? (NT / PK) * SPR : NS;
            auto tap_of = [&](int st) -> int { return RAG ? (st / SPR) * PK + 2 * (st % SPR) : st / KH32; };
            auto paired = [&](int st) -> bool { return RAG && (st % SPR) < PK / 2; };
            auto toff_of = [&](int st) -> int {
                const int tap = tap_of(st), half = RAG ? 0 : st % KH32;
                return (((tap / (SS::KW * SS::KH)) * SHH + (tap / SS::KW) % SS::KH) * SHW + tap % SS::KW) * VS + half * 64;
            };
            int abP[RAG ? WPX : 1];
            if constexpr (RAG) {
                const int pd = (l4 >= 2) ? (SS::KW > 1 ? VS : SHW * VS) - 32 : 0;
#pragma unroll
                for (int pi = 0; pi < WPX; ++pi) abP[pi] = abase[pi] + pd;
            }
            auto ab_of = [&](int pi, int st) -> int { return paired(st) ? abP[RAG ? pi : 0] : abase[pi]; };
            h8_t afA[HA > 0 ? HA : 1], afB[WPX - HA];
#pragma unroll
            for (int pi = 0; pi < HA; ++pi) afA[pi] = *(const h8_t*)(hb + ab_of(pi, 0) + toff_of(0));
#if defined(CS_NO_ILV)
            constexpr bool ILV = false;
#elif defined(CS_ILV_ALL)
            constexpr bool ILV = (WPX >= 2);
#elif defined(CS_ILV_128)
            constexpr bool ILV = (WPX == 8 && WVP == 2) || (WPX == 8 && WCH == 2 && WVP == 1);
#else
            constexpr bool ILV = (WPX == 8 && WVP == 2);
#endif
#pragma unroll
// ... 63 lines not shown
        auto it_next_chunk = [&](It& it) {
            ++it.cc; it.nh = it.cc < cc_hi ? chunk_nhalf(it.cc) : 1; it.tap = 0; it.half = j0;
            while (it.half >= it.nh) { it.half -= it.nh; ++it.tap; }
        };
        auto it_advance = [&](It& it) {
            it.half += SKS;
            while (it.half >= it.nh) { it.half -= it.nh; ++it.tap; }
        };
        It P;
        it_init(P);
        long last_off = 0;
        auto wload = [&](u4_t (&dst)[WCH]) {
            while (P.cc < cc_hi && it_chunk_done(P)) it_next_chunk(P);
            if (P.cc < cc_hi) { last_off = (long)((P.cc * KH32 + P.half) * ntaps + P.tap) * wstep; it_advance(P); }
            const half_t* src = wlane + last_off;
            wfrag_load<0>(dst[0], src);
            if constexpr (WCH > 1) wfrag_load<ep_frag_row(EP_PAIR, 1) * 64>(dst[1], src);
            if constexpr (WCH > 2) wfrag_load<ep_frag_row(EP_PAIR, 2) * 64>(dst[2], src);
            if constexpr (WCH > 3) wfrag_load<ep_frag_row(EP_PAIR, 3) * 64>(dst[3], src);
            if constexpr (WCH > 4) wfrag_load<0>(dst[4], src + ep_frag_row(EP_PAIR, 4) * 32);
        };

        u4_t wr[PFD][WCH];
    #pragma unroll
        for (int i = 0; i < PFD; ++i) wload(wr[i]);

        TL_STAMP(1);
        stage_halo(0, cc_lo * CK);
        __syncthreads();
        TL_STAMP(2);
        if (DB && cc_lo + 1 < cc_hi) stage_halo(1, (cc_lo + 1) * CK);
        int cur = 0;
        It C;
        it_init(C);
        int ckw = C.tap % KW, ckh = (C.tap / KW) % KH, ckd = C.tap / (KW * KH), ctap = C.tap;
        const unsigned char* hb = smem;
        bool done = false;
        while (!done) {
    #pragma unroll
            for (int i = 0; i < PFD; ++i) {
                while (!done && it_chunk_done(C)) {
                    if (C.cc + 1 >= cc_hi) { done = true; break; }
                    if (DB) {
                        __syncthreads();
                        if (C.cc + 2 < cc_hi) stage_halo(cur, (C.cc + 2) * CK);
                        cur ^= 1;
                    } else {
                        __syncthreads();
                        stage_halo(0, (C.cc + 1) * CK);
                        __syncthreads();
                    }
                    it_next_chunk(C);
                    ctap = C.tap; ckw = ctap % KW; ckh = (ctap / KW) % KH; ckd = ctap / (KW * KH);
                    hb = smem + (size_t)cur * HV * VS;
                }
                if (done) break;
                while (ctap < C.tap) { ++ctap; if (++ckw == KW) { ckw = 0; if (++ckh == KH) { ckh = 0; ++ckd; } } }
                const int toff = ((ckd * HH + ckh) * HW + ckw) * VS + C.half * 64;
                h8_t af[WPX];
    #pragma unroll
                for (int pi = 0; pi < WPX; ++pi) af[pi] = *(const h8_t*)(hb + abase[pi] + toff);
                wait_vmcnt_le<WCH*(PFD - 1)>();
                __builtin_amdgcn_sched_barrier(0);
    #pragma unroll
                for (int ci = 0; ci < WCH; ++ci)
    #pragma unroll
                    for (int pi = 0; pi < WPX; ++pi)
                        acc[ci][pi] = __builtin_amdgcn_mfma_f32_16x16x32_f16(__builtin_bit_cast(h8_t, wr[i][ci]), af[pi], acc[ci][pi], 0, 0, 0);
                __builtin_amdgcn_sched_barrier(0);
                wload(wr[i]);
                it_advance(C);
            }
        }
    }

    if constexpr (ST == 0) {
        wait_vmcnt_le<0>();
        __builtin_amdgcn_sched_barrier(0);
    }

    constexpr bool EP_HEAVY = (MODE == MODE_PIXSHUF) || (WCH == 1) || (ST == 15) || (ST == 0);
    constexpr bool KWSUM = !SK && MODE == MODE_STD && WCH == 5 && WPX == 8 && WVP == 2 && (ST == 8 || ST == 9);
    TL_STAMP(3);
    if constexpr (!SK) {
        if (p.sk_out) {
            const long mtot = (long)p.N * p.D * p.H * p.W;
#pragma unroll
            for (int pi = 0; pi < WPX; ++pi) {
                int m = wpx * WPX * 16 + pi * 16 + l15p;
                const int w = (tw << lgTW) + (m & mW); m >>= lgTW;
                const int h = (th << lgTH) + (m & mH); m >>= lgTH;
                const int d = (td << lgTD) + (m & mD); m >>= lgTD;
                const int n = tn * TN + m;
                if (n >= p.N) continue;
                const long pos = (((long)n * p.D + d) * p.H + h) * p.W + w;
#pragma unroll
                for (int ci = 0; ci < WCH; ++ci)
                    *(f4_t*)(p.sk_out + ((long)blockIdx.z * mtot + pos) * p.Cout_pad + ep_chan(EP_PAIR, 1, n0 + wch * WCH * 16, ci, l4)) = acc[ci][pi];
            }
        } else if (XSK && p.xs_w) {
            if constexpr (XSK) {
                __syncthreads();
                float* part = (float*)smem;
                const int cw0 = n0 + wch * 64;
                h8_t wsA[4][2];
#pragma unroll
                for (int of = 0; of < 4; ++of)
#pragma unroll
                    for (int q = 0; q < 2; ++q)
                        wsA[of][q] = *(const h8_t*)(p.xs_w + ((long)((cw0 >> 5) + q) * 64 + of * 16 + l15) * 32 + l4 * 8);
                float gb[2][8], mu[2][8], rs[2][8];
#pragma unroll
                for (int q = 0; q < 2; ++q) {
                    const int cb = cw0 + q * 32 + l4 * 8;
#pragma unroll
                    for (int j = 0; j < 8; j += 4) {
                        const float4 b4 = p.bias ? *(const float4*)(p.bias + cb + j) : make_float4(0.f, 0.f, 0.f, 0.f);
                        gb[q][j] = b4.x; gb[q][j + 1] = b4.y; gb[q][j + 2] = b4.z; gb[q][j + 3] = b4.w;
                        const float4 q0 = *(const float4*)(p.stats + ((long)tn * p.Cout + cb + j) * 2);
                        const float4 q1 = *(const float4*)(p.stats + ((long)tn * p.Cout + cb + j) * 2 + 4);
                        mu[q][j] = q0.x; rs[q][j] = q0.y; mu[q][j + 1] = q0.z; rs[q][j + 1] = q0.w;
                        mu[q][j + 2] = q1.x; rs[q][j + 2] = q1.y; mu[q][j + 3] = q1.z; rs[q][j + 3] = q1.w;
                    }
                }
                const int rsh = p.res_shift;
                const half_t* xrow = (const half_t*)p.res.p + (long)tn * p.res.sN + cw0 + l4 * 8;
                const int ow = (tw << lgTW) + l15p, oh0 = th << lgTH;
                auto xfetch = [&](int pi, int q) -> u4_t {
                    return *(const u4_t*)(xrow + (long)((oh0 + pi) >> rsh) * p.res.sH + (long)(ow >> rsh) * p.res.sW + q * 32);
                };
                u4_t xr[2] = {xfetch(0, 0), xfetch(0, 1)};
                const int oc = wave * 16 + l4 * 4;
                const bool has_b = p.xs_res.p != nullptr && oc < p.xs_cout;
                auto bfetch = [&](int pi) -> h4_t {
                    return *(const h4_t*)((const half_t*)p.xs_res.p + ((long)tn * p.xs_res.sN + (long)(oh0 + pi) * p.xs_res.sH + (long)ow * p.xs_res.sW + oc));
                };
                h4_t br = (h4_t){0, 0, 0, 0};
                if (has_b) br = bfetch(0);
#pragma unroll
                for (int pi = 0; pi < WPX; ++pi) {
                    u4_t xn[2] = {xr[0], xr[1]};
                    h4_t bn = br;
                    if (pi + 1 < WPX) { xn[0] = xfetch(pi + 1, 0); xn[1] = xfetch(pi + 1, 1); if (has_b) bn = bfetch(pi + 1); }
                    h8_t hB[2];
#pragma unroll
                    for (int q = 0; q < 2; ++q) {
                        const h8_t xh = __builtin_bit_cast(h8_t, xr[q]);
                        unsigned pk[4];
#pragma unroll
                        for (int j = 0; j < 8; j += 2) {
                            float v2[2];
#pragma unroll
                            for (int e = 0; e < 2; ++e) {
                                const int jj = j + e;
                                const float g = acc[2 * q + (jj >> 2)][pi][jj & 3] + gb[q][jj];
                                v2[e] = (((float)xh[jj] - mu[q][jj]) * rs[q][jj]) * (1.f + g);
                            }
                            pk[j >> 1] = ep_pk(v2[0], v2[1]);
                        }
                        u4_t t4; t4[0] = pk[0]; t4[1] = pk[1]; t4[2] = pk[2]; t4[3] = pk[3];
                        hB[q] = __builtin_bit_cast(h8_t, t4);
                    }
                    float* pb = part + (size_t)(pi & 1) * (4 * 4 * 64 * 4);
#pragma unroll
                    for (int of = 0; of < 4; ++of) {
                        f4_t a = (f4_t){0.f, 0.f, 0.f, 0.f};
                        a = __builtin_amdgcn_mfma_f32_16x16x32_f16(wsA[of][0], hB[0], a, 0, 0, 0);
// ... 81 lines not shown
                float* const gbase = p.kw_out + ((((long)tn * p.D + (td << lgTD) + wpx * WPX) * p.H + (th << lgTH)) * p.nTW + tw) * 176;
                const long gslice = (long)p.H * p.nTW * 176;
#pragma unroll
                for (int pi = 0; pi < WPX; ++pi) {
#pragma unroll
                    for (int ci = 0; ci < WCH; ++ci) *(f4_t*)(buf + l15p * 160 + wch * (WCH * 16) + ci * 16 + l4 * 4) = acc[ci][pi];
                    __syncthreads();
#pragma unroll
                    for (int q = 0; q < 3; ++q) {
                        if (q * 128 + th128 < 352) {
                            f4_t v;
#pragma unroll
                            for (int e = 0; e < 4; ++e) v[e] = buf[offA[q * 4 + e]] + buf[offB[q * 4 + e]];
                            *(f4_t*)(gbase + pi * gslice + goff[q]) = v;
                        }
                    }
                    __syncthreads();
                }
            }
        } else {
        constexpr int EP_WPX = WPX;
        const int ep_wpx = wpx;
        auto& ep_acc = acc;
        CONV_EPILOGUE()
        }
    } else {
        __syncthreads();
        float* red = (float*)smem;
#pragma unroll
        for (int ci = 0; ci < WCH; ++ci)
#pragma unroll
            for (int pi = 0; pi < WPX; ++pi)
#pragma unroll
                for (int r = 0; r < 4; ++r) red[((wave * WCH * WPX + ci * WPX + pi) * 4 + r) * 64 + lane] = acc[ci][pi][r];
        __syncthreads();
        constexpr int EP_WPX = 2;
        const int ep_wpx = wave;
        f4_t ep_acc[WCH][EP_WPX];
#pragma unroll
        for (int ci = 0; ci < WCH; ++ci)
#pragma unroll
            for (int q = 0; q < EP_WPX; ++q) {
                const int pi = wave * EP_WPX + q;
#pragma unroll
                for (int r = 0; r < 4; ++r) {
                    float s = 0.f;
#pragma unroll
                    for (int w = 0; w < 4; ++w) s += red[((w * WCH * WPX + ci * WPX + pi) * 4 + r) * 64 + lane];
                    ep_acc[ci][q][r] = s;
                }
            }
        CONV_EPILOGUE()
    }
    if (!ASMRK || !has_next) break;
    ++p_j;
    }
#ifdef CS_TIMELINE
    TL_STAMP(4);
    asm volatile("s_waitcnt vmcnt(0)" ::: "memory");
    TL_STAMP(5);
    const unsigned long long tl_real5 = __builtin_amdgcn_s_memrealtime();
    if (p.tl && lane == 0) {
        const long wi = ((long)blockIdx.y * gridDim.x + blockIdx.x) * 4 + wave;
        if (wi < p.tl_cap) {
            unsigned hwid, xcc;
            asm volatile("s_getreg_b32 %0, hwreg(HW_REG_HW_ID)" : "=s"(hwid));
            asm volatile("s_getreg_b32 %0, hwreg(HW_REG_XCC_ID)" : "=s"(xcc));
            unsigned long long* o = p.tl + wi * 12;
#pragma unroll
            for (int i = 0; i < 8; ++i) o[i] = tl_t[i];
            o[8] = tl_real0; o[9] = tl_real5; o[10] = hwid; o[11] = xcc;
        }
    }
#endif
}

static inline int lgS_of(const ConvParams& p) { return p.lgTW + p.lgTH + p.lgTD; }
template <int CK, int WPX, int WCH, int WVP, int WVC, int MODE, bool SK, int ST>
static int launch_halo_st(const ConvParams& p, hipStream_t st)
{
    constexpr int BM = SK ? WPX * 16 : WPX * 16 * WVP, BN = WCH * 16 * WVC;
    constexpr int PAD = halo_pad<CK, WPX, WCH, WVP, ST, MODE>(), HI = halo_hi<ST, PAD>();
    constexpr int SLP = CK / 8 + PAD, VS = SLP * 16;
    if (p.Cout_pad % BN != 0) { cs_set_error("conv_halo: Cout_pad %d not a multiple of the channel tile %d", p.Cout_pad, BN); return -1; }
    {
        const long in_span = (long)(p.N - 1) * p.in_sN + (long)(p.D - 1) * p.in_sD + (long)(p.H - 1) * p.in_sH + (long)(p.W - 1) * p.in_sW +
                             p.Cin + (p.cg > 0 ? (long)(p.nchunks / p.cg) * p.in_sG : 0);
        if (in_span >= (1L << 31)) { cs_set_error("conv_halo: the input spans 2^31 elements or more (32-bit in-tensor offsets)"); return -1; }
        if (p.in_sD >= (1L << 23) || p.in_sH >= (1L << 23) || p.in_sW >= (1L << 23)) {
            cs_set_error("conv_halo: an input axis stride of 2^23 elements or more (24-bit multiplies in the addressing)");
            return -1;
        }
        if (ep_check_extents(p, "conv_halo")) return -1;
    }
    constexpr bool heavy_ok = (MODE == MODE_PIXSHUF) || (WCH == 1) || (ST == 15) || (ST == 0);
    if ((!heavy_ok && p.act0 >= ACT_SIGMOID) || p.act1 >= ACT_SIGMOID) {
        cs_set_error("conv_halo: this tile configuration carries no sigmoid / GELU epilogue (act0 %d, act1 %d)", p.act0, p.act1);
        return -1;
    }
    if (p.inD != p.D) { cs_set_error("conv_halo: depth-collapsing convs are not supported"); return -1; }
    if (p.pool_hw && !p.sk_out) {
        using SSL = StaticShape<ST>;
        constexpr bool poolk = ST != 0 && !SK && MODE == MODE_STD && WCH == 2 && SSL::KD == 3 && SSL::KH == 3 && SSL::KW == 3 && (SSL::LW == 3 || SSL::LW == 2) && SSL::LH >= 1;
        constexpr bool poolk2 = halo_pool2d<CK, WPX, WCH, WVP, MODE, SK, ST>();
        if (!(poolk || poolk2) || p.res.p || p.out1.p || p.pixscale || p.stat_out || p.out0_f32 || !p.out0.p || p.sk_out || p.ep_general || (p.H & 1) || (p.W & 1) ||
            p.Cout % 8 || p.Cout != p.Cout_pad || (1 << lgS_of(p)) != BM || ((unsigned long long)p.out0.p & 15ull) ||
            ((p.out0.sN | p.out0.sD | p.out0.sH | p.out0.sW) & 7)) {
            cs_set_error("conv_halo: pool_hw (AvgPool(1,2,2) in the epilogue) needs a static 3x3x3 tile of 8 or 4 columns with two channel fragments per wave or a 2-D 16x8 tile with 32-channel chunks, fp16 out0 only, every packed channel real");
            return -1;
        }
    }
    if (p.spmul) {
        if (MODE != MODE_STD || SK || !p.res.p || p.res_f32 || !p.stats || p.out1.p || p.pixscale || p.stat_out || p.pool_hw || p.sk_out || p.kw_out ||
            (1 << lgS_of(p)) != BM) {
            cs_set_error("conv_halo: spmul (out0 = act0(IN(res) (1 + conv))) is a mode-STD epilogue with an fp16 res, stats, one output and tiles within one sample");
            return -1;
        }
    }
    if (p.xs_w) {
        constexpr bool xsk = ST == 1 && !SK && MODE == MODE_STD && CK == 64 && WCH == 4 && WPX == 8 && WVP == 1;
        if (!xsk || !p.spmul || p.out0.p || p.Cout != 256 || p.Cout_pad != 256 || p.xs_cout < 4 || p.xs_cout > 64 || p.xs_cout % 4 || !p.xs_out.p || p.act0 != ACT_NONE ||
            p.lgTW != 4 || p.lgTH != 3 || ((unsigned long long)p.res.p & 15ull) || ((p.res.sN | p.res.sH | p.res.sW) & 7) || ((unsigned long long)p.xs_w & 15ull) ||
            ((unsigned long long)p.xs_out.p & 7ull) || ((p.xs_out.sN | p.xs_out.sH | p.xs_out.sW) & 3) ||
            (p.xs_res.p && (((unsigned long long)p.xs_res.p & 7ull) || ((p.xs_res.sN | p.xs_res.sH | p.xs_res.sW) & 3)))) {
            cs_set_error("conv_halo: xs_w (conv_s inside the spmul epilogue) needs the 128 x 256 tile kernel, 256 modulated channels, no out0, at most 64 shortcut channels");
            return -1;
        }
    }
    if (p.kw_out) {
        constexpr bool kwsum = !SK && MODE == MODE_STD && WCH == 5 && WPX == 8 && WVP == 2 && (ST == 8 || ST == 9);
        if (!kwsum || p.Cout_pad != 160 || p.lgTH != 3 || !((p.lgTW == 1 && p.lgTD == 4) || (p.lgTW == 2 && p.lgTD == 3)) || p.sk_out || p.W % (1 << p.lgTW) ||
            p.nTN != p.N) {
            cs_set_error("conv_halo: kw_out is the mask conv's epilogue (7x7x1 taps, 160 packed channels, 2x8x16 or 4x8x8 tiles of one sample)");
            return -1;
        }
    }
    const int lgS = p.lgTW + p.lgTH + p.lgTD;
    if ((1 << lgS) > BM) { cs_set_error("conv_halo: spatial tile exceeds BM"); return -1; }
    if (MODE == MODE_SPADE && (1 << lgS) != BM) { cs_set_error("conv_halo: SPADE launches must tile within one sample"); return -1; }
    if (MODE == MODE_SPADE && p.res_f32) { cs_set_error("conv_halo: the tensor a SPADE launch modulates is fp16"); return -1; }
    if (p.ragged) {
        constexpr bool ragk = (CK == 32) && (WPX == 8) && (ST == 7 || ST == 8 || ST == 9) && MODE == MODE_STD;
        if (!ragk || SK || p.Cin % 32 != 16 || p.sk_out || p.hilo || p.cg > 0) {
            cs_set_error("conv_halo: paired-tap weights (ragged) need the 256-position 32-channel static kernels and Cin %% 32 == 16");
            return -1;
        }
    }
    if (p.wslot && (1 << lgS) != BM) { cs_set_error("conv_halo: per-sample weight sets need tiles within one sample"); return -1; }
    if (p.cg > 0 && CK != 32 && (!(ST == 15 || (ST == 0 && WCH != 4)) || (p.cg & 1) || (p.in_sG & 63) || p.KD * p.KH * p.KW != 1)) {
        cs_set_error("conv_halo: grouped input channels run 32-channel chunks (64-channel chunks: 1x1 convs with an even number of 32-channel pieces per group)");
        return -1;
    }
    const int TN = BM >> lgS;
    const long HV = (long)TN * ((1 << p.lgTD) + p.KD - 1) * ((1 << p.lgTH) + p.KH - 1) * ((1 << p.lgTW) + p.KW - 1);
    const int nck = (p.Cin + CK - 1) / CK;
    constexpr bool big = (BM == 256 && WCH == 5);
#ifndef CS_NO_ASMRING
    constexpr bool asmr = WCH == 5 && WPX == 8 && WVP == 2 && (ST == 7 || ST == 8 || ST == 9) && MODE == MODE_STD && !SK;
#else
    constexpr bool asmr = false;
#endif
    const bool db = nck > 1 && (asmr ? 2 * HI * 4096 <= 160 * 1024 : 2 * HV * VS <= (big || (WCH == 4 && PAD == 2) ? 128 : 64) * 1024) && HV * SLP <= 256 * HI;
    size_t lds = (size_t)(db ? 2 : 1) * HV * VS + 16;
    ConvParams kp = p;
    if (asmr && db) {
        lds = (size_t)2 * HI * 4096;
        const long span = (long)(p.inD - 1) * p.in_sD + (long)((p.H - 1) >> p.up_shift) * p.in_sH + (long)((p.W - 1) >> p.up_shift) * p.in_sW + p.Cin + 32;
        if (span >= (1L << 30) || p.cg > 0 || p.hilo || (1 << lgS) != BM) {
            cs_set_error("conv_halo: the 256 x 160 tiles address one sample of the input through a buffer of less than 2^31 bytes (no grouped / split-precision input)");
            return -1;
        }
        kp.in_sample_bytes = (unsigned)(span * 2);
    }
    kp.persist_total = 0;
    if (SK && lds < (size_t)4 * WCH * WPX * 4 * 64 * sizeof(float)) lds = (size_t)4 * WCH * WPX * 4 * 64 * sizeof(float);
    if (p.xs_w && lds < (size_t)32768) lds = 32768;
    if (lds > 160 * 1024) { cs_set_error("conv_halo: halo of %ld voxels does not fit LDS", HV); return -1; }
    dim3 grid((unsigned)(p.nTW * p.nTH * p.nTD * p.nTN), (unsigned)(p.Cout_pad / BN));
    if (p.hilo && (ST == 0 || CK != 32 || nck != 3 || db || p.sk_out)) {
        cs_set_error("conv_halo: the hi/lo split-precision mode needs a static-shape 32-channel kernel with three single-buffered chunks");
        return -1;
    }
    if (p.nphase) {
        if (SK || !halo_phase_group<WCH, ST>() || p.nphase < 1 || p.nphase > 4 || p.sk_out || p.kw_out || p.xs_w || p.persist_total < 0) { cs_set_error("conv_halo: bad grouped launch (%d phases)", p.nphase); return -1; }
        if (p.res.p || p.stat_out || p.pixscale || p.spmul || p.pool_hw) { cs_set_error("conv_halo: a grouped launch carries out0 / out1 only (no res / statistics / pixel scale / spmul / pooling)"); return -1; }
        for (int z = 0; z < p.nphase; ++z)
            if (p.ph_ooff[z] % 8u) { cs_set_error("conv_halo: output offset of phase %d (%u elements) is not a multiple of 8 (16-byte stores)", z, p.ph_ooff[z]); return -1; }
        grid.z = (unsigned)p.nphase;
    }
    if (p.sk_out) {
        if (SK || p.sk_splits < 1 || p.sk_splits > nck || p.xcd_map == 2) { cs_set_error("conv_halo: bad split-K launch (%d splits, %d chunks)", p.sk_splits, nck); return -1; }
        grid.z = (unsigned)p.sk_splits;
    }
    if (p.xcd_map == 2) grid = dim3(grid.x * grid.y, 1, grid.z);
    hipError_t e;
    {
        const unsigned long long umax = (unsigned long long)grid.x * grid.y;
        const unsigned ds[4] = {(unsigned)(p.Cout_pad / BN), (unsigned)p.nTW, (unsigned)p.nTH, (unsigned)p.nTD};
        unsigned mg[4];
        for (int i = 0; i < 4; ++i) {
            if (ds[i] == 0 || umax * ds[i] >= (1ull << 32)) { cs_set_error("conv_halo: launch of %llu workgroups / tile count %u too large", umax, ds[i]); return -1; }
            mg[i] = ds[i] == 1 ? 0u : (unsigned)((1ull << 32) / ds[i]) + 1u;
        }
        kp.mg_ncb = mg[0]; kp.mg_tw = mg[1]; kp.mg_th = mg[2]; kp.mg_td = mg[3];
    }
#ifdef CS_TIMELINE
    kp.tl = g_cs_tl; kp.tl_cap = g_cs_tl_cap;
#endif
    if (asmr && db && p.persist_total != 0 && !p.sk_out && !p.nphase) {
        const unsigned total = grid.x * grid.y;
        kp.persist_total = (int)total;
        grid = dim3(total < 256u ? (total + 7u) & ~7u : 256u, 1);
    }
    if (db) {
        auto k = conv_halo_kernel<CK, WPX, WCH, WVP, WVC, MODE, true, SK, ST>;
        if (lds > 64 * 1024) {
            e = hipFuncSetAttribute((const void*)k, hipFuncAttributeMaxDynamicSharedMemorySize, (int)lds);
            if (e != hipSuccess) { cs_set_error("conv_halo: opting into %zu bytes of LDS failed: %s", lds, hipGetErrorString(e)); return -1; }
        }
        hipLaunchKernelGGL(k, grid, dim3(256), lds, st, kp);
    } else {
        auto k = conv_halo_kernel<CK, WPX, WCH, WVP, WVC, MODE, false, SK, ST>;
        if (lds > 64 * 1024) {
            e = hipFuncSetAttribute((const void*)k, hipFuncAttributeMaxDynamicSharedMemorySize, (int)lds);
            if (e != hipSuccess) { cs_set_error("conv_halo: opting into %zu bytes of LDS failed: %s", lds, hipGetErrorString(e)); return -1; }
        }
        hipLaunchKernelGGL(k, grid, dim3(256), lds, st, kp);
    }
    e = hipGetLastError();
    if (e != hipSuccess) { cs_set_error("conv_halo launch: %s", hipGetErrorString(e)); return -1; }
    return 0;
}
```

canonswap_amd/csrc/engine.hip:

```cpp
#include "common.h"
#include "../../include/canonswap_hip.h"

#include <cstdarg>
#include <cstdio>
#include <cstdlib>
#include <cstring>
#include <initializer_list>
#include <map>
#include <string>
#include <vector>

static thread_local char g_err[1024] = "";
void cs_set_error(const char* fmt, ...)
{
    va_list ap;
    va_start(ap, fmt);
    vsnprintf(g_err, sizeof(g_err), fmt, ap);
    va_end(ap);
}
extern "C" const char* cs_last_error(void) { return g_err; }
extern "C" int cs_abi_version(void) { return CS_ABI_VERSION; }

#define TRY(x) do { if ((x) != 0) return -1; } while (0)

// ... 134 lines not shown

int get_conv(cs_engine* e, const std::string& n, int Cin, int Cout_pad, int Cout, int KD, int KH, int KW, int bias_len,
             double macs, ConvL* L)
{
    const int nch = (Cin + 31) / 32;
    const void* p;
    TRY(need(e, n + ".w", (size_t)nch * KD * KH * KW * Cout_pad * 32 * sizeof(half_t), &p));
    L->w = (const half_t*)p;
    L->b = nullptr;
    if (bias_len > 0) { TRY(need(e, n + ".b", (size_t)bias_len * sizeof(float), &p)); L->b = (const float*)p; }
    L->Cin = Cin; L->Cout_pad = Cout_pad; L->Cout = Cout; L->KD = KD; L->KH = KH; L->KW = KW;
    L->macs_per_pos = macs; L->ragged = false;
    L->name = n;
    return 0;
}

int get_affine(cs_engine* e, const std::string& n, int len, Affine* a)
{
    const void* p;
    TRY(need(e, n + ".s", (size_t)len * 4, &p)); a->s = (const float*)p;
    TRY(need(e, n + ".t", (size_t)len * 4, &p)); a->t = (const float*)p;
    return 0;
}

int get_f32(cs_engine* e, const std::string& n, int len, const float** out)
{
    const void* p;
    TRY(need(e, n, (size_t)len * 4, &p));
    *out = (const float*)p;
    return 0;
}

TDesc td(void* p, long sN, long sD, long sH, long sW) { return TDesc{p, sN, sD, sH, sW}; }
TDesc nhwc(void* p, int H, int W, int C) { return td(p, (long)H * W * C, 0, (long)W * C, C); }
TDesc hwdc3(void* p) { return td(p, VOL, FC, (long)FW * FD * FC, (long)FD * FC); }
TDesc hwdc2(void* p) { return td(p, VOL, 0, (long)FW * FD * FC, (long)FD * FC); }
TDesc dhwc(void* p, int D, int H, int W, int stride) { return td(p, (long)D * H * W * stride, (long)H * W * stride, (long)W * stride, stride); }

int ilog2(int v) { int l = 0; while ((1 << l) < v) ++l; return l; }

struct ConvCall {
    ConvParams p;
    int cfg = -1, mode = MODE_STD;
    int hcfg = -1;
    int stat_nblk = 0;
    bool cg_ck64 = false;
    double macs_per_pos = 0;
    const char* name = "";
};

ConvCall mk(const ConvL& L, const void* in, TDesc ind, int N, int D, int H, int W, int up_shift = 0)
{
    ConvCall c;
    memset(&c.p, 0, sizeof(c.p));
    ConvParams& p = c.p;
    p.in = (const half_t*)in;
    p.zero = cs_zero_page();
    p.in_sN = ind.sN; p.in_sD = ind.sD; p.in_sH = ind.sH; p.in_sW = ind.sW;
    p.N = N; p.D = D; p.H = H; p.W = W; p.inD = D;
    p.Cin = L.Cin; p.nchunks = (L.Cin + 31) / 32; p.up_shift = up_shift;
    p.KD = L.KD; p.KH = L.KH; p.KW = L.KW; p.PD = L.KD / 2; p.PH = L.KH / 2; p.PW = L.KW / 2;
    p.wgt = L.w; p.Cout_pad = L.Cout_pad; p.Cout = L.Cout; p.ragged = L.ragged;
    p.bias = L.b;
    p.ps_stride = 1;
    c.macs_per_pos = L.macs_per_pos;
    c.name = L.name.c_str();
    return c;
}

void set_tile(ConvParams& p, int BM, int prefW, int prefH)
{
    int tw = p.W < prefW ? p.W : prefW;
    int th = p.H < prefH ? p.H : prefH;
    while (tw * th > BM) th >>= 1;
    int tdd = BM / (tw * th);
    if (tdd > p.D) tdd = p.D;
    int tn = BM / (tw * th * tdd);
    p.lgTW = ilog2(tw); p.lgTH = ilog2(th); p.lgTD = ilog2(tdd);
    p.nTW = p.W / tw; p.nTH = p.H / th; p.nTD = p.D / tdd; p.nTN = (p.N + tn - 1) / tn;
}

int cfg_v32() { return CFG_H_256x32; }

constexpr int HALO_PERSIST = 1;
constexpr int XCD_MAP = 2;

int pick_halo_cfg(const ConvParams& p, int mode)
{
    const int Cout_pad = p.Cout_pad;
    if (mode == MODE_PIXSHUF) return CFG_H_256x16;
    if (mode == MODE_TBLEND && Cout_pad % 256 == 0 && p.KD == 1 && p.KH == 3 && p.KW == 3 && p.W >= 16 && p.H >= 8 && p.Cin % 32 == 0 &&
        (long)p.N * p.H * p.W >= 3 * 4096) return CFG_H_128x256;
    if (mode == MODE_SPADE && Cout_pad % 256 == 0 && p.KD == 1 && p.KH == 3 && p.KW == 3 && p.W >= 16 && p.H >= 8 && p.Cin % 64 == 0 &&
        (long)p.N * p.H * p.W >= 3 * 4096) return CFG_H_128x256;
    if ((mode == MODE_STD || mode == MODE_STDSTAT) && Cout_pad % 256 == 0 && p.KD == 1 && p.KH == 3 && p.KW == 3 &&
        p.W >= 16 && p.H >= 8 && p.Cin % 64 == 0 && (long)p.N * p.H * p.W >= 3 * 4096) return CFG_H_128x256;
    if (Cout_pad % 128 == 0) {
        const long tiles = ((long)p.N * p.D * p.H * p.W + 127) / 128;
        const bool k33 = p.KH == 3 && p.KW == 3, k11 = p.KD == 1 && p.KH == 1 && p.KW == 1 && mode == MODE_STD;
        if ((mode == MODE_STD || mode == MODE_STDSTAT) && (k33 || k11) && tiles * (Cout_pad / 128) <= 128)
            return CFG_H_128x64;
        if (k11 && tiles * (Cout_pad / 128) < 256) return CFG_H_128x64;
        return CFG_H_128x128;
    }
    if (Cout_pad == 64 && (mode == MODE_STD || mode == MODE_STDSTAT) && p.KD == 1 && p.KH == 3 && p.KW == 3 && p.Cin % 64 == 0 && p.cg == 0 &&
        p.H % 16 == 0 && p.W % 16 == 0 && p.H >= 128 && !p.sk_out) return CFG_H_256x64;
    if (Cout_pad % 64 == 0) return CFG_H_128x64;
    if (Cout_pad % 32 == 0) return CFG_H_128x32;
    return CFG_H_128x16;
}

int amax_after(cs_engine* e, const struct ConvCall& c, hipStream_t st);

constexpr int VOL32_MINB = 3;
bool vol32_enabled() { static const bool on = [] { const char* s = getenv("CANONSWAP_VOL32"); return !s || atoi(s) != 0; }(); return on; }
bool vol32_xf() { static const bool on = [] { const char* s = getenv("CANONSWAP_VOL32_XF"); return !s || atoi(s) != 0; }(); return on && vol32_enabled(); }

int go(cs_engine* e, ConvCall& c, hipStream_t st, int prefW = 0, int prefH = 0)
{
    const int nph = c.p.nphase > 0 ? c.p.nphase : 1;
    const double fl = 2.0 * c.macs_per_pos * (double)c.p.N * c.p.D * c.p.H * c.p.W * nph;
    e->flops += fl;
    {
        double ksteps = (double)c.p.nchunks * c.p.KD * c.p.KH * c.p.KW;
        if (c.p.ragged) {
            const int NT = c.p.KD * c.p.KH * c.p.KW, PK = c.p.KW > 1 ? c.p.KW : c.p.KH;
            ksteps -= NT - (NT / PK) * (PK / 2 + PK % 2);
        }
        e->flops_exec += 2.0 * (double)c.p.N * c.p.D * c.p.H * c.p.W * c.p.Cout_pad * 32.0 * ksteps * nph;
    }
    if (vol32_enabled() && vol32_supported(c.p) && (c.p.N >= VOL32_MINB || c.p.stat_out || c.p.xf_kind)) {
        if (e->latency_mode && c.p.stat_out) c.p.v32_srows = 2;
        c.stat_nblk = vol32_stat_nblk(c.p);
        TRY(e->run(0, st, [&] { return launch_vol32(c.p, st); }, c.name, fl));
        return amax_after(e, c, st);
    }
    if (c.p.xf_kind) { cs_set_error("%s: transform staging needs the vol32 kernel", c.name); return -1; }
    static const int wide_on = [] { const char* s = getenv("CANONSWAP_WIDE"); return s ? atoi(s) : 1; }();
    if (wide_on && !e->latency_mode && c.hcfg < 0 && (c.mode != MODE_SPADE || wide_on >= 2)) {
        if (conv_wide_supported(c.p, c.mode) && (long)c.p.N * (c.p.H / 16) * (c.p.W / 16) * (c.p.Cout_pad / 256) >= 512) {
            c.stat_nblk = (c.p.W / 16) * (c.p.H / 8) * 2;
            TRY(e->run(0, st, [&] { return launch_conv_wide(c.p, c.mode, st); }, c.name, fl));
            return amax_after(e, c, st);
        }
    }
    if (e->latency_mode && c.hcfg < 0 && conv_lat_supported(c.p, c.mode) &&
        (long)c.p.N * (c.p.H / 8) * (c.p.W / 16) * (c.p.Cout_pad / (c.mode == MODE_TBLEND ? 128 : 64)) <= 256) {
        c.stat_nblk = (c.p.W / 16) * (c.p.H / 8) * 2;
        TRY(e->run(0, st, [&] { return launch_conv_lat(c.p, c.mode, st); }, c.name, fl));
        return amax_after(e, c, st);
    }
    if (c.p.inD == c.p.D) {
        const int hcfg = c.hcfg >= 0 ? c.hcfg : pick_halo_cfg(c.p, c.mode);
        const int BM = (hcfg == CFG_H_256x32 || hcfg == CFG_H_256x16 || hcfg == CFG_H_256x160 || hcfg == CFG_H_256x64) ? 256 : 128;
        const bool is3d = c.p.KD > 1;
        if (!prefW) { prefW = is3d ? 8 : 16; prefH = is3d ? 8 : BM / 16; }
        set_tile(c.p, BM, prefW, prefH);
        {
            int wave_px = 64;
            if (hcfg == CFG_H_128x32 || hcfg == CFG_H_128x16 || hcfg == CFG_H_SK128x32) wave_px = 32;
            c.stat_nblk = c.p.nTW * c.p.nTH * c.p.nTD * (BM / wave_px);
        }
        const bool spade_ck32 = c.mode == MODE_SPADE && c.p.Cout_pad % 256 != 0;
        const bool k11 = c.p.KD == 1 && c.p.KH == 1 && c.p.KW == 1;
        const bool cg64 = c.cg_ck64 && k11 && c.p.cg > 0 && !(c.p.cg & 1) && c.p.Cin % 64 == 0 && c.mode == MODE_STD;
        const int ck = (!is3d && c.p.Cin % 64 == 0 && (c.p.cg == 0 || cg64) && !spade_ck32) ? 64 : 32;
        c.p.xcd_map = XCD_MAP;
        c.p.persist_total = HALO_PERSIST;
        {
            const bool sk_on = e->latency_mode;
            const int bn = hcfg == CFG_H_128x256 ? 256 : hcfg == CFG_H_128x128 ? 128 : hcfg == CFG_H_128x64 || hcfg == CFG_H_256x64 ? 64 :
                           hcfg == CFG_H_128x160 || hcfg == CFG_H_256x160 ? 160 : hcfg == CFG_H_128x16 || hcfg == CFG_H_256x16 ? 16 : 32;
            const long wgs = (long)c.p.nTW * c.p.nTH * c.p.nTD * c.p.nTN * (c.p.Cout_pad / bn);
            const int nck = (c.p.Cin + ck - 1) / ck;
            const long mtot = (long)c.p.N * c.p.D * c.p.H * c.p.W;
            const bool plain = c.mode == MODE_STD && !c.p.res.p && !c.p.pixscale && !c.p.out1.p && !c.p.stat_out && !c.p.s2 &&
                               c.p.act0 <= ACT_SIGMOID && c.p.out0.p && hcfg != CFG_H_SK128x32 && c.p.Cout % 4 == 0 && !c.p.spmul && !c.p.nphase &&
                               (!c.p.pool_hw || (!c.p.out0_f32 && !(c.p.H & 1) && !(c.p.W & 1)));
            constexpr int sk_maxwg = 64, sk_fill = 512;
            if (sk_on && plain && wgs <= sk_maxwg && nck >= 4 && e->sk_buf) {
                int splits = (int)(sk_fill / wgs);
                if (splits > nck) splits = nck;
                if (splits > 16) splits = 16;
                while (splits > 1 && (size_t)splits * mtot * c.p.Cout_pad > e->sk_cap) --splits;
                if (splits >= 2) {
                    c.p.sk_out = e->sk_buf; c.p.sk_splits = splits; c.p.xcd_map = 0;
                    TRY(e->run(0, st, [&] { return launch_conv_halo(c.p, hcfg, ck, c.mode, st); }, c.name, fl));
                    return e->run(1, st, [&] { return launch_splitk_finish(c.p, st); }, "splitk_finish");
                }
            }
        }
        TRY(e->run(0, st, [&] { return launch_conv_halo(c.p, hcfg, ck, c.mode, st); }, c.name, fl));
        return amax_after(e, c, st);
    }
    cs_set_error("%s: no conv_halo launch for this convolution (depth-collapsing convs are not supported)", c.name);
    return -1;
}

float* stats_slot(cs_engine* e);

int amax_after(cs_engine* e, const ConvCall& c, hipStream_t st)
{
    static const bool on = [] { const char* s = getenv("CANONSWAP_AMAX"); return s && atoi(s) != 0; }();
    if (!on || !e->prof || e->recs.empty()) return 0;
    if (!e->amax_dev) { if (e->alloc(&e->amax_dev, (size_t)4096)) return -1; }
    if (e->amax_n >= 4096) return 0;
    const ConvParams& p = c.p;
    const bool o0 = p.out0.p && !p.out0_f32 && c.mode != MODE_PIXSHUF, o1 = p.out1.p != nullptr;
    if (!o0 && !o1) return 0;
    const int slot = e->amax_n++;
    hipError_t r = hipMemsetAsync(e->amax_dev + slot, 0, sizeof(unsigned), st);
    if (r != hipSuccess) { cs_set_error("amax memset: %s", hipGetErrorString(r)); return -1; }
    if (o0) TRY(launch_absmax16((const half_t*)p.out0.p, p.out0, p.N, p.D, p.H, p.W, p.Cout, e->amax_dev + slot, st));
    if (o1) TRY(launch_absmax16((const half_t*)p.out1.p, p.out1, p.N, p.D, p.H, p.W, p.Cout, e->amax_dev + slot, st));
    for (auto it = e->recs.rbegin(); it != e->recs.rend(); ++it) if (it->fam == 0) { it->amax_slot = slot; break; }
    return 0;
}

int go_stats(cs_engine* e, ConvCall& c, int C, long P, float** slot, hipStream_t st, int prefW = 0, int prefH = 0)
{
    c.p.stat_out = e->stats_part;
    TRY(go(e, c, st, prefW, prefH));
    float* s = stats_slot(e);
    *slot = s;
    const int nblk = c.stat_nblk, N = c.p.N;
    if ((long)nblk * C * 2 > 262144) { cs_set_error("%s: statistics partials do not fit (%d blocks x %d)", c.name, nblk, C); return -1; }
    return e->run(1, st, [&] { return launch_chan_stats_finish(e->stats_part, nblk, N, C, 1.0 / (double)P, 1e-5f, s, st); }, "chan_stats_finish");
}

float* stats_slot(cs_engine* e)
{
    float* p = e->stats_pool + (e->stats_next % e->stats_slots) * e->stats_slot_floats;
    e->stats_next++;
    return p;
}

int do_stats(cs_engine* e, const void* x, int is_f32, int B, long P, int C, float** out, hipStream_t st)
{
    float* slot = stats_slot(e);
    *out = slot;
    return e->run(1, st, [&] { return launch_chan_stats(x, is_f32, B, P, C, 1e-5f, e->stats_part, slot, st); }, "chan_stats");
}

bool vol32_fused_on() { static const bool on = [] { const char* s = getenv("CANONSWAP_VOL32_FUSED"); return !s || atoi(s) != 0; }(); return on && vol32_enabled(); }

int run_resblocks3d(cs_engine* e, cs_engine::RB3* rb, int B, int* cur, hipStream_t st)
{
    if (vol32_fused_on()) {
        for (int i = 0; i < 6; ++i) {
            const int nxt = (*cur + 1) % 3;
            ResBlock3dCall c;
            c.a = e->va[i & 1]; c.x = e->vs[*cur]; c.out0 = e->vs[nxt]; c.out1 = e->va[(i + 1) & 1];
            c.sN = VOL; c.sH = (long)FW * FD * FC; c.sW = (long)FD * FC;
            c.w1 = rb[i].c1.w; c.w2 = rb[i].c2.w; c.b1 = rb[i].c1.b; c.b2 = rb[i].c2.b;
            c.s2 = nullptr; c.t2 = nullptr; c.act1 = ACT_NONE; c.slope1 = 0.f;
            if (i < 5) { c.s2 = rb[i].post.s; c.t2 = rb[i].post.t; c.act1 = ACT_RELU; }
            c.N = B; c.H = FH; c.W = FW;
            const double fl = 2.0 * (rb[i].c1.macs_per_pos + rb[i].c2.macs_per_pos) * (double)B * VOX;
            e->flops += fl;
            e->flops_exec += 2.0 * 2.0 * (double)B * VOX * 32 * 32.0 * 27;
// ... 31 lines not shown
    TRY(e->run(1, st, [&] { return launch_conv_first(img, e->first_w, e->first_b, e->f_t0, B, IMG, IMG, st); }, "conv_first"));
    e->flops += 2.0 * 3 * 64 * 9 * (double)B * IMG * IMG;
    ConvCall d0 = mk(e->f_down0, e->f_t0, nhwc(nullptr, 256, 256, 64), B, 1, 256, 256);
    d0.p.act0 = ACT_RELU; wsplit_in(d0, 64);
    d0.p.pool_hw = 1; d0.p.out0 = nhwc(e->f_p0, 128, 128, 128);
    TRY(go(e, d0, st));
    ConvCall d1 = mk(e->f_down1, e->f_p0, nhwc(nullptr, 128, 128, 128), B, 1, 128, 128);
    d1.p.act0 = ACT_RELU; wsplit_in(d1, 128);
    d1.p.pool_hw = 1; d1.p.out0 = nhwc(e->f_p1, 64, 64, 256);
    TRY(go(e, d1, st));
    *cur = 0;
    ConvCall s = mk(e->f_second, e->f_p1, nhwc(nullptr, 64, 64, 256), B, 1, 64, 64);
    s.p.out0 = hwdc2(e->vs[0]); s.p.out0_f32 = 1;
    s.p.out1 = hwdc2(e->va[0]); s.p.s2 = e->f_pre0.s; s.p.t2 = e->f_pre0.t; s.p.act1 = ACT_RELU; wsplit_in(s, 256);
    TRY(go(e, s, st));
    return run_resblocks3d(e, e->f_rb, B, cur, st);
}

bool warp_fused() { static const bool on = [] { const char* s = getenv("CANONSWAP_WARP_FUSED"); return !s || atoi(s) != 0; }(); return on; }

static bool dec_phases_deep() { static const bool on = [] { const char* s = getenv("CANONSWAP_DEC_PHASES_DEEP"); return !s || atoi(s) != 0; }(); return on; }

int run_dense_motion(cs_engine* e, int B, const float* feat, const float* kp_d, const float* kp_s, hipStream_t st,
                     const float* warp_in = nullptr, float* warp_o32 = nullptr, half_t* warp_o16 = nullptr, bool want_deform = false,
                     bool shared_feat = false, bool shared_kps = false)
{
    TRY(e->run(1, st, [&] { return launch_dm_compress(feat, e->cmp_w, e->cmp_b, e->dm_comp, shared_feat ? 1 : B, FD, FH, FW, st); }, "dm_compress"));
    e->flops += 2.0 * 32 * 4 * VOX * B;
    TRY(e->run(1, st, [&] { return launch_dm_sparse(e->dm_comp, kp_d, kp_s, e->dm_l[0] + 32, 144, B, FD, FH, FW, st, shared_feat, shared_kps); }, "dm_sparse"));
    static const int cout[5] = {64, 128, 256, 512, 1024};
    static const int skip_off[6] = {32, 64, 128, 256, 512, 0};
    for (int i = 0; i < 5; ++i) {
        const int S = 64 >> i;
        ConvCall c = mk(e->w_enc[i], e->dm_l[i] + skip_off[i], dhwc(nullptr, FD, S, S, DM_LW[i]), B, FD, S, S);
        c.p.act0 = ACT_RELU;
        c.p.out0 = dhwc(e->dm_pre, FD, S, S, cout[i]);
        if (i == 0) c.hcfg = CFG_H_256x64;
        TDesc o = dhwc(e->dm_l[i + 1] + skip_off[i + 1], FD, S / 2, S / 2, DM_LW[i + 1]);
        c.p.pool_hw = 1; c.p.out0 = o;
        TRY(go(e, c, st));
    }
    for (int i = 0; i < 5; ++i) {
        const int lv = 5 - i, S = 64 >> (lv - 1), Si = S / 2;
        ConvCall c = mk(e->w_dec[i], e->dm_l[lv], dhwc(nullptr, FD, Si, Si, DM_LW[lv]), B, FD, S, S, 1);
        c.p.act0 = ACT_RELU;
        c.p.out0 = dhwc(e->dm_l[lv - 1], FD, S, S, DM_LW[lv - 1]);
        if (i >= 3 || (!e->latency_mode && dec_phases_deep())) {
            const int lwo = DM_LW[lv - 1];
            static const bool grouped = [] { const char* s = getenv("CANONSWAP_PHASE_GROUP"); return !s || atoi(s) != 0; }();
            if (!grouped) {
                for (int ab = 0; ab < 4; ++ab) {
                    const int a = ab >> 1, b = ab & 1;
                    ConvCall q1 = mk(e->w_dec_p[i][ab], e->dm_l[lv], dhwc(nullptr, FD, Si, Si, DM_LW[lv]), B, FD, Si, Si);
                    q1.p.PH = a == 0; q1.p.PW = b == 0;
                    q1.p.act0 = ACT_RELU;
                    q1.p.out0 = td(e->dm_l[lv - 1] + ((long)a * S + b) * lwo, (long)FD * S * S * lwo, (long)S * S * lwo, 2L * S * lwo, 2L * lwo);
                    if (i == 4) { q1.hcfg = CFG_H_256x32; TRY(go(e, q1, st, 4, 4)); }
                    else TRY(go(e, q1, st));
                }
                continue;
            }
            ConvCall q = mk(e->w_dec_p[i][0], e->dm_l[lv], dhwc(nullptr, FD, Si, Si, DM_LW[lv]), B, FD, Si, Si);
            q.p.act0 = ACT_RELU;
            q.p.out0 = td(e->dm_l[lv - 1], (long)FD * S * S * lwo, (long)S * S * lwo, 2L * S * lwo, 2L * lwo);
            q.p.nphase = 4;
            for (int ab = 0; ab < 4; ++ab) {
                const int a = ab >> 1, b = ab & 1;
                q.p.ph_wofs[ab] = (long)(((intptr_t)e->w_dec_p[i][ab].w - (intptr_t)e->w_dec_p[i][0].w) / (intptr_t)sizeof(half_t));
                q.p.ph_ooff[ab] = (unsigned)(((long)a * S + b) * lwo);
                q.p.ph_PH[ab] = a == 0; q.p.ph_PW[ab] = b == 0;
            }
            q.p.PH = 1; q.p.PW = 1;
            static const char* const pn[5] = {"W.dec0.p", "W.dec1.p", "W.dec2.p", "W.dec3.p", "W.dec4.p"};
            q.name = pn[i];
            if (i == 4) { q.hcfg = CFG_H_256x32; TRY(go(e, q, st, 4, 4)); }
            else TRY(go(e, q, st));
            continue;
        }
        if (i == 4) { c.hcfg = CFG_H_256x32; TRY(go(e, c, st, 4, 4)); continue; }
        TRY(go(e, c, st));
    }
    ConvCall t = mk(e->w_tail, e->dm_l[0], dhwc(nullptr, FD, 64, 64, 144), B, FD, 64, 64);
    t.p.act0 = ACT_RELU; t.p.out0 = dhwc(e->dm_pred, FD, 64, 64, 144);
    t.hcfg = CFG_H_256x160;
    TRY(go(e, t, st));
    ConvCall m = mk(e->w_mask, e->dm_pred, dhwc(nullptr, FD, 64, 64, 144), B, FD, 64, 64);
    m.p.kw_out = e->dm_logits;
    m.hcfg = CFG_H_256x160;
    TRY(go(e, m, st, 4, 8));
    if (warp_in && warp_fused()) {
        TRY(e->run(2, st, [&] { return launch_dm_softmax_warp(e->dm_logits, e->mask_b, kp_d, kp_s, warp_in, warp_o32, warp_o16, want_deform ? e->dm_deform : nullptr, B, FD, FH, FW, st, shared_feat, shared_kps); },
                   "dm_softmax_warp"));
    } else {
        TRY(e->run(1, st, [&] { return launch_dm_softmax(e->dm_logits, e->mask_b, kp_d, kp_s, e->dm_deform, B, FD, FH, FW, st, shared_kps); }, "dm_softmax"));
        if (warp_in) TRY(e->run(2, st, [&] { return launch_grid_sample(warp_in, e->dm_deform, warp_o32, warp_o16, B, FD, FH, FW, st, shared_feat); }, "grid_sample"));
    }
    if (!e->latency_mode) {
        ConvCall oc = mk(e->w_occ49, e->dm_pred, td(nullptr, (long)FD * 4096 * 144, 0, 64L * 144, 144), B, 1, 64, 64);
        oc.p.cg = 5; oc.p.cg_cin = 144; oc.p.in_sG = 4096L * 144;
        oc.p.out0 = nhwc(e->dm_occpart, 64, 64, 64); oc.p.out0_f32 = 1;
        oc.hcfg = CFG_H_128x64;
        TRY(go(e, oc, st));
        TRY(e->run(1, st, [&] { return launch_occ_finish49(e->dm_occpart, e->occ_b, e->dm_occ, B, 64, 64, st); }, "occ_finish"));
        return 0;
    }
    ConvCall oc = mk(e->w_occ, e->dm_pred, td(nullptr, (long)FD * 4096 * 144, 0, 64L * 144, 144), B, 1, 64, 64);
    oc.p.cg = 5; oc.p.cg_cin = 144; oc.p.in_sG = 4096L * 144;
    oc.p.out0 = nhwc(e->dm_occpart, 64, 64, 16); oc.p.out0_f32 = 1;
    oc.hcfg = e->latency_mode ? CFG_H_128x32 : CFG_H_SK128x32;
    TRY(go(e, oc, st));
    TRY(e->run(1, st, [&] { return launch_occ_finish(e->dm_occpart, e->occ_b, e->dm_occ, B, 64, 64, st); }, "occ_finish"));
    return 0;
}

int run_warp_out(cs_engine* e, int B, const half_t* vol16, const float* occ, hipStream_t st)
{
    ConvCall t3 = mk(e->w_third, vol16, hwdc2(nullptr), B, 1, 64, 64);
    t3.p.act0 = ACT_LRELU; t3.p.slope0 = 0.01f;
    t3.p.out0 = nhwc(e->w_t3, 64, 64, 256);
    TRY(go(e, t3, st));
    ConvCall f4 = mk(e->w_fourth, e->w_t3, nhwc(nullptr, 64, 64, 256), B, 1, 64, 64);
    f4.p.pixscale = occ;
    f4.p.out0 = nhwc(e->seg16, 64, 64, 256);
    return go(e, f4, st);
}

int t_slots(cs_engine* e, int B, const int* slots, bool* mixed, hipStream_t st)
{
    *mixed = false;
    for (int b = 0; b < B; ++b) {
        if (slots[b] < 0 || slots[b] >= MAX_SLOTS) { cs_set_error("cs_swap: identity slot %d outside [0, %d)", slots[b], MAX_SLOTS); return -1; }
        if (!e->slot_set[slots[b]]) { cs_set_error("cs_swap: cs_set_identity has not been called for slot %d", slots[b]); return -1; }
        *mixed |= slots[b] != slots[0];
    }
    if (*mixed) {
        if (e->slot_cur.size() != (size_t)B || memcmp(e->slot_cur.data(), slots, sizeof(int) * B) != 0) {
            int* stage = e->slot_pin + (size_t)(e->slot_ring++ % 16) * e->maxB;
            memcpy(stage, slots, sizeof(int) * B);
            hipError_t r = hipMemcpyAsync(e->slot_dev, stage, sizeof(int) * B, hipMemcpyHostToDevice, st);
            if (r != hipSuccess) { cs_set_error("slot upload: %s", hipGetErrorString(r)); return -1; }
            e->slot_cur.assign(slots, slots + B);
        }
    }
    return 0;
}

int t_layer(cs_engine* e, int layer, int B, const int* slots, bool mixed, const half_t* in, const float* res32, float* tmask, half_t* out16,
            float* out32, hipStream_t st)
{
    TLayer& L = e->t_l[layer];
    {
        const double mfl = 2.0 * L.mask.macs_per_pos * (double)B * 4096;
        e->flops += mfl; e->flops_exec += mfl;
        TRY(e->run(0, st, [&] { return launch_t_mask(in, L.mask.w, L.mask.b, tmask, B, 64, 64, st); }, L.mask.name.c_str(), mfl));
    }
    ConvCall fc = mk(L.fused, in, hwdc2(nullptr), B, 1, 64, 64);
    fc.mode = MODE_TBLEND;
    if (mixed) { fc.p.wgt = L.wset[0]; fc.p.wofs = L.wofs; fc.p.wslot = e->slot_dev; }
    else fc.p.wgt = L.wset[slots[0]];
    fc.p.Cout = 512;
    fc.p.bias = L.bias;
    fc.p.pixscale = tmask; fc.p.ps_stride = 4;
    if (layer % 2 == 0) {
        fc.p.act0 = ACT_RELU;
        fc.p.out0 = hwdc2(out16);
    } else {
        fc.p.res = hwdc2((void*)res32); fc.p.res_f32 = 1;
// ... 926 lines not shown
    hipStream_t st = (hipStream_t)stream;
    return e->run(1, st, [&] { return launch_face_masks(logits, B, C, h, w, scale, valid_bits, masks, labels, st); }, "face_masks");
}

extern "C" int cs_profile_begin(cs_engine* e)
{
    if (!e) { cs_set_error("null engine"); return -1; }
    e->prof = true; e->recs.clear(); e->evnext = 0; e->flops = 0; e->flops_exec = 0; e->amax_n = 0;
    return 0;
}

extern "C" int cs_profile_end(cs_engine* e, double ms[3], long counts[3], double* flops)
{
    if (!e) { cs_set_error("null engine"); return -1; }
    CS_CHECK_HIP(hipDeviceSynchronize());
    ms[0] = ms[1] = ms[2] = 0; counts[0] = counts[1] = counts[2] = 0;
    FILE* csv = nullptr;
    if (const char* path = getenv("CANONSWAP_PROFILE_CSV")) csv = fopen(path, "w");
    std::vector<unsigned> amax((size_t)e->amax_n);
    if (e->amax_n) CS_CHECK_HIP(hipMemcpy(amax.data(), e->amax_dev, sizeof(unsigned) * e->amax_n, hipMemcpyDeviceToHost));
    if (csv) fprintf(csv, e->amax_n ? "family,label,ms,gflop,fp16_amax\n" : "family,label,ms,gflop\n");
    for (auto& r : e->recs) {
        float t = 0;
        CS_CHECK_HIP(hipEventElapsedTime(&t, r.a, r.b));
        ms[r.fam] += t; counts[r.fam]++;
        if (csv && e->amax_n) {
            float am = -1.f;
            if (r.amax_slot >= 0) memcpy(&am, &amax[r.amax_slot], 4);
            if (am >= 0) fprintf(csv, "%d,%s,%.5f,%.4f,%.6g\n", r.fam, r.label.c_str(), t, r.flops / 1e9, am);
            else fprintf(csv, "%d,%s,%.5f,%.4f,\n", r.fam, r.label.c_str(), t, r.flops / 1e9);
        } else if (csv) fprintf(csv, "%d,%s,%.5f,%.4f\n", r.fam, r.label.c_str(), t, r.flops / 1e9);
    }
    if (csv) fclose(csv);
    if (flops) *flops = e->flops;
    e->prof = false; e->recs.clear(); e->evnext = 0;
    return 0;
}

extern "C" int cs_set_latency_mode(cs_engine* e, int on)
{
    if (!e) { cs_set_error("null engine"); return -1; }
    e->latency_mode = on != 0;
    return 0;
}

extern "C" int cs_profile_exec_flops(cs_engine* e, double* flops)
{
    if (!e || !flops) { cs_set_error("cs_profile_exec_flops: bad arguments"); return -1; }
    *flops = e->flops_exec;
    return 0;
}

extern "C" int cs_op_conv(const cs_conv_desc* d, void* stream)
{
    ConvCall c;
    memset(&c.p, 0, sizeof(c.p));
    ConvParams& p = c.p;
    p.in = (const half_t*)d->in; p.zero = cs_zero_page(); p.in_sN = d->in_sN; p.in_sD = d->in_sD; p.in_sH = d->in_sH; p.in_sW = d->in_sW;
    p.N = d->N; p.D = d->D; p.H = d->H; p.W = d->W; p.inD = d->D; p.Cin = d->Cin; p.nchunks = (d->Cin + 31) / 32; p.up_shift = d->up_shift;
    p.KD = d->KD; p.KH = d->KH; p.KW = d->KW; p.PD = d->KD / 2; p.PH = d->KH / 2; p.PW = d->KW / 2;
    p.wgt = (const half_t*)d->wgt; p.Cout_pad = d->Cout_pad; p.Cout = d->Cout;
    p.bias = d->bias; p.bias2 = d->bias2; p.act0 = d->act0; p.slope0 = d->slope0;
    p.res = td((void*)d->res, d->res_sN, d->res_sD, d->res_sH, d->res_sW); p.res_f32 = d->res_f32; p.res_shift = d->res_shift;
    p.pixscale = d->pixscale; p.ps_stride = d->ps_stride ? d->ps_stride : 1;
    p.out0 = td(d->out0, d->out0_sN, d->out0_sD, d->out0_sH, d->out0_sW); p.out0_f32 = d->out0_f32;
    p.s2 = d->s2; p.t2 = d->t2; p.act1 = d->act1; p.slope1 = d->slope1;
    p.out1 = td(d->out1, d->out1_sN, d->out1_sD, d->out1_sH, d->out1_sW);
    p.stats = d->stats;
    p.hilo = d->hilo; p.stat_out = d->stat_out; p.pool_hw = d->pool_hw;
    if (d->xf_kind) {
        p.xf_kind = d->xf_kind;
        p.xf_y = td((void*)d->xf_y, d->out0_sN, d->out0_sD, d->out0_sH, d->out0_sW);
        p.xf_res = td((void*)d->xf_res, d->out0_sN, d->out0_sD, d->out0_sH, d->out0_sW);
        p.xf_out = td((void*)d->xf_out, d->out0_sN, d->out0_sD, d->out0_sH, d->out0_sW);
        p.xf_stats = d->xf_stats; p.xf_gamma = d->xf_gamma; p.xf_beta = d->xf_beta; p.xf_slope = d->xf_slope;
    }
    c.mode = d->mode;
    if (d->mode == 5) { c.mode = MODE_STD; p.spmul = 1; }
    if (d->cfg == CFG_VOL32) return launch_vol32(p, (hipStream_t)stream);
    if (d->cfg == CFG_WIDE) return launch_conv_wide(p, c.mode, (hipStream_t)stream);
    if (d->cfg == CFG_LAT) return launch_conv_lat(p, c.mode, (hipStream_t)stream);
    if (d->cfg >= 10 || d->cfg == -2) {
        const int hcfg = d->cfg >= 10 ? d->cfg : pick_halo_cfg(p, c.mode);
        const int BM = (hcfg == CFG_H_256x32 || hcfg == CFG_H_256x16 || hcfg == CFG_H_256x160 || hcfg == CFG_H_256x64) ? 256 : 128;
        const bool is3d = p.KD > 1;
        set_tile(p, BM, d->tile_w ? d->tile_w : (is3d ? 8 : 16), d->tile_h ? d->tile_h : (is3d ? 8 : BM / 16));
        const int ck = d->ck ? d->ck : ((!is3d && p.Cin % 64 == 0) ? 64 : 32);
        p.xcd_map = d->xcd_map > 0 ? d->xcd_map - 1 : XCD_MAP;
        p.persist_total = HALO_PERSIST;
        p.ragged = d->ragged;
        p.ep_general = d->ep_general;
        return launch_conv_halo(p, hcfg, ck, c.mode, (hipStream_t)stream);
    }
    cs_set_error("cs_op_conv: cfg %d is not a conv_halo configuration (the conv_igemm cross-check kernel lives in the test-only library)", d->cfg);
    return -1;
}

extern "C" int cs_op_resblock3d(const void* a, const float* x, float* out0, void* out1, int N, int H, int W, const void* w1, const void* w2,
                                const float* b1, const float* b2, const float* s2, const float* t2, int act1, float slope1, void* stream)
{
    ResBlock3dCall c;
    c.a = (const half_t*)a; c.x = x; c.out0 = out0; c.out1 = (half_t*)out1;
    c.sN = (long)H * W * 512; c.sH = (long)W * 512; c.sW = 512;
    c.w1 = (const half_t*)w1; c.w2 = (const half_t*)w2; c.b1 = b1; c.b2 = b2; c.s2 = s2; c.t2 = t2; c.act1 = act1; c.slope1 = slope1;
    c.N = N; c.H = H; c.W = W;
    return launch_vol32_fused(c, (hipStream_t)stream);
}

extern "C" int cs_op_t_mask(const void* x, const void* wpacked, const float* bias, float* tmask, int N, int H, int W, void* stream)
{
    return launch_t_mask((const half_t*)x, (const half_t*)wpacked, bias, tmask, N, H, W, (hipStream_t)stream);
}

extern "C" int cs_op_t_style(const float* id, const float* fc, float* style, int nlayers, void* stream)
{
    if (!id || !fc || !style || nlayers < 1) { cs_set_error("cs_op_t_style: bad arguments"); return -1; }
    return launch_t_style(id, fc, style, nlayers, (hipStream_t)stream);
}

extern "C" int cs_op_t_modulate(const float* wraw, const float* style, void* packed, void* stream)
{
    if (!wraw || !style || !packed) { cs_set_error("cs_op_t_modulate: bad arguments"); return -1; }
    return launch_t_modulate(wraw, style, (half_t*)packed, 0, (hipStream_t)stream);
}

extern "C" int cs_op_t_read(cs_engine* e, int layer, int slot, int which, void* dst, void* stream)
{
    if (!e || !e->finalized) { cs_set_error("cs_op_t_read: engine not finalized"); return -1; }
    if (!dst) { cs_set_error("cs_op_t_read: null destination"); return -1; }
    if (layer < 0 || layer >= 14) { cs_set_error("cs_op_t_read: layer %d outside [0, 14)", layer); return -1; }
    if (slot < 0 || slot >= MAX_SLOTS) { cs_set_error("cs_op_t_read: identity slot %d outside [0, %d)", slot, MAX_SLOTS); return -1; }
    if (!e->slot_set[slot]) { cs_set_error("cs_op_t_read: cs_set_identity has not been called for slot %d", slot); return -1; }
    DevGuard guard(e->dev);
    if (which == CS_T_WSET) return copy_dd(dst, e->t_l[layer].wset[slot], (size_t)144 * 1024 * 32 * sizeof(half_t), (hipStream_t)stream);
    if (which == CS_T_STYLE) return copy_dd(dst, e->style + layer * 512, 512 * sizeof(float), (hipStream_t)stream);
    cs_set_error("cs_op_t_read: no buffer %d", which);
    return -1;
}

extern "C" int cs_op_t_layer(cs_engine* e, int layer, int B, const int* slots, const void* in16, const float* res32, float* tmask_out, void* out16,
                             float* out32, void* stream)
{
    ENTER(e, B);
    if (layer < 0 || layer >= 14) { cs_set_error("cs_op_t_layer: layer %d outside [0, 14)", layer); return -1; }
    const bool conv2 = layer % 2 == 1;
    if (!slots || !in16 || !tmask_out || !out16 || (conv2 && (!res32 || !out32)) || (!conv2 && (res32 || out32))) {
        cs_set_error("cs_op_t_layer: bad arguments (conv2 layers take res32 and out32, conv1 layers neither)");
        return -1;
    }
    hipStream_t st = (hipStream_t)stream;
    bool mixed = false;
    TRY(t_slots(e, B, slots, &mixed, st));
    return t_layer(e, layer, B, slots, mixed, (const half_t*)in16, res32, tmask_out, (half_t*)out16, out32, st);
}

extern "C" int cs_op_pair_ragged(void* w, int Cout_pad, int nchunks, int KD, int KH, int KW, void* stream)
{
    return launch_pair_ragged((half_t*)w, Cout_pad, nchunks, KD, KH, KW, (hipStream_t)stream);
}

extern "C" int cs_op_grid_sample3d(const float* in_hwdc, const float* grid, float* out32, void* out16, int N, int D, int H, int W,
                                   void* stream)
{
    return launch_grid_sample(in_hwdc, grid, out32, (half_t*)out16, N, D, H, W, (hipStream_t)stream);
}

extern "C" long cs_op_chan_stats_partial_floats(int N, long P, int C) { return chan_stats_partial_floats(N, P, C); }
// ... 97 lines not shown
```

Measured before the change: 545.4 frames/s.

## Add 256x144 halo conv variant that skips padded output rows for tail conv

Adds a CFG_H_256x144 form of the 256x160 ASMR 3x3x3 conv kernel that computes only the 144 real output channels instead of all 160 padded ones. Each wave keeps four 16-channel fragments plus half of a ninth fragment, and the ninth fragment's pixel blocks are split across the two channel waves using a rotated pixel order. The dense-motion tail conv uses it by default, with an environment switch to fall back. The aim is to drop about 10% of the MFMA work on that conv. In exchange the register layout, epilogue paths and load scheduling become more complex, and the variant only accepts the plain bias-plus-activation epilogue.

```diff
diff --git a/canonswap_amd/_lib.py b/canonswap_amd/_lib.py
--- a/canonswap_amd/_lib.py
+++ b/canonswap_amd/_lib.py
@@ -211,7 +211,7 @@
 
 def _isa_check_wide(obj_dir: str, objdump: str) -> dict:
     seen = _isa_check_ring(obj_dir, objdump, "conv_wide.o", r"\S*conv_wide_kernel\S*", 18 * 64)
-    seen.update(_isa_check_ring(obj_dir, objdump, "conv_halo_g1.o", r"_Z16conv_halo_kernelILi32ELi8ELi5ELi2ELi2ELi0ELb1ELb0ELi[789]E\S*", None))
+    seen.update(_isa_check_ring(obj_dir, objdump, "conv_halo_g1.o", r"_Z16conv_halo_kernelILi32ELi8ELi5ELi2ELi2ELi0ELb1ELb0ELi(?:[789]|18)E\S*", None))
     return seen
 
 
diff --git a/canonswap_amd/csrc/common.h b/canonswap_amd/csrc/common.h
--- a/canonswap_amd/csrc/common.h
+++ b/canonswap_amd/csrc/common.h
@@ -16,6 +16,7 @@
        CFG_H_128x160 = 18 ,
        CFG_H_256x160 = 19 ,
        CFG_H_256x64 = 20 ,
+       CFG_H_256x144 = 21 ,
        CFG_VOL32 = 30 , CFG_WIDE = 31 ,
        CFG_LAT = 32  };
 
diff --git a/canonswap_amd/csrc/conv_epilogue.h b/canonswap_amd/csrc/conv_epilogue.h
--- a/canonswap_amd/csrc/conv_epilogue.h
+++ b/canonswap_amd/csrc/conv_epilogue.h
@@ -203,6 +203,9 @@
 #ifndef EP_SLICE_FENCE
 #define EP_SLICE_FENCE
 #endif
+#ifndef EP_BLK_OF
+#define EP_BLK_OF(pi) (ep_wpx * EP_WPX + (pi))
+#endif
 #ifndef EP_FG
 #define EP_FG 8
 #endif
@@ -242,7 +245,7 @@
 _Pragma("unroll") \
         for (int g = 0; g < EP_G; ++g) { \
             int bw, bh, bd, bn; \
-            { int t = (ep_wpx * EP_WPX + (PG0) + g) << 4; bw = t & mW; t >>= lgTW; bh = t & mH; t >>= lgTH; bd = t & mD; t >>= lgTD; bn = t; } \
+            { int t = EP_BLK_OF((PG0) + g) << 4; bw = t & mW; t >>= lgTW; bh = t & mH; t >>= lgTH; bd = t & mD; t >>= lgTD; bn = t; } \
             if (!EPFAST && ep_nb + ep_ln + bn >= p.N) continue; \
             if (ep_has_ps) ep_ps2[BI][g] = p.pixscale[ep_lane_ps + (unsigned)((((bn * p.D + bd) * p.H + bh) * p.W + bw) * p.ps_stride)]; \
             if (ep_fetch) { \
@@ -352,7 +355,7 @@
         if (pi == 1) EP_TL(7); \
         if (pi > 0 && pi % EP_SG == 0) { EP_STAT_FLUSH(pi / EP_SG - 1) } \
         int bw, bh, bd, bn; \
-        { int t = (ep_wpx * EP_WPX + pi) << 4; bw = t & mW; t >>= lgTW; bh = t & mH; t >>= lgTH; bd = t & mD; t >>= lgTD; bn = t; } \
+        { int t = EP_BLK_OF(pi) << 4; bw = t & mW; t >>= lgTW; bh = t & mH; t >>= lgTH; bd = t & mD; t >>= lgTD; bn = t; } \
         if (!EPFAST && ep_nb + ep_ln + bn >= p.N) continue; \
         float ps = 1.f; \
         if (ep_has_ps) ps = EP_PF ? ep_ps[g] : p.pixscale[ep_lane_ps + (unsigned)((((bn * p.D + bd) * p.H + bh) * p.W + bw) * p.ps_stride)]; \
diff --git a/canonswap_amd/csrc/conv_halo.hip b/canonswap_amd/csrc/conv_halo.hip
--- a/canonswap_amd/csrc/conv_halo.hip
+++ b/canonswap_amd/csrc/conv_halo.hip
@@ -78,6 +78,16 @@
         if (p.KD == 7 && p.lgTW == 2) return launch_halo_cfg<32, 8, 5, 2, 2, MODE_STD, false, 9>(p, st);
         if (p.KD == 7) return launch_halo_cfg<32, 8, 5, 2, 2, MODE_STD, false, 8>(p, st);
         return launch_halo_cfg<32, 8, 5, 2, 2, MODE_STD, false, 7>(p, st);
+    }
+    if (cfg == CFG_H_256x144) {
+        using SS = StaticShape<18>;
+        if (mode == MODE_STDSTAT) { cs_set_error("conv_halo: the 256 x 144 tile's epilogue is bias + activation into one out0; this launch asks for statistics"); return -1; }
+        if (mode != MODE_STD || ck != 32 || p.KD != SS::KD || p.KH != SS::KH || p.KW != SS::KW || p.lgTW != SS::LW || p.lgTH != SS::LH || p.lgTD != SS::LD) {
+            cs_set_error("conv_halo: the 256 x 144 tile runs mode-STD 3x3x3 convs on 8x8x4 tiles with 32-channel chunks (mode %d, %dx%dx%d taps, tile 2^%d x 2^%d x 2^%d, chunk %d)",
+                         mode, p.KD, p.KH, p.KW, p.lgTW, p.lgTH, p.lgTD, ck);
+            return -1;
+        }
+        return launch_halo_st<32, 8, 5, 2, 2, MODE_STD, false, 18>(p, st);
     }
     if (cfg == CFG_H_128x160 && mode == MODE_STD && ck == 32) {
         if (stv == 4) return launch_halo_cfg<32, 4, 5, 2, 2, MODE_STD, false, 4>(p, st);
diff --git a/canonswap_amd/csrc/conv_halo_kernel.h b/canonswap_amd/csrc/conv_halo_kernel.h
--- a/canonswap_amd/csrc/conv_halo_kernel.h
+++ b/canonswap_amd/csrc/conv_halo_kernel.h
@@ -13,6 +13,7 @@
 #define EP_MLIN_V EP_MLIN_K
 #define EP_O1ONLY_V EP_O1ONLY_K
 #define EP_O0_EXTRA_V ep_o0_extra
+#define EP_BLK_OF(pi) (ep_wpx * EP_WPX + ((pi) ^ ep_prot))
 #include "conv_epilogue.h"
 
 typedef unsigned int u4_t __attribute__((ext_vector_type(4)));
@@ -37,6 +38,8 @@
 #define TL_STAMP(i) do { } while (0)
 #endif
 
+constexpr bool halo_t256(int ST) { return ST == 7 || ST == 8 || ST == 9 || ST == 18; }
+constexpr bool halo_t144(int ST) { return ST == 18; }
 template <int ST> struct StaticShape { static constexpr int KD = 0, KH = 0, KW = 0, LW = 0, LH = 0, LD = 0; };
 template <> struct StaticShape<1> { static constexpr int KD = 1, KH = 3, KW = 3, LW = 4, LH = 3, LD = 0; };
 template <> struct StaticShape<2> { static constexpr int KD = 3, KH = 3, KW = 3, LW = 3, LH = 3, LD = 1; };
@@ -46,6 +49,7 @@
 template <> struct StaticShape<6> { static constexpr int KD = 7, KH = 7, KW = 1, LW = 1, LH = 3, LD = 3; };
 template <> struct StaticShape<7> { static constexpr int KD = 3, KH = 3, KW = 3, LW = 3, LH = 3, LD = 2; };
 template <> struct StaticShape<8> { static constexpr int KD = 7, KH = 7, KW = 1, LW = 1, LH = 3, LD = 4; };
+template <> struct StaticShape<18> { static constexpr int KD = 3, KH = 3, KW = 3, LW = 3, LH = 3, LD = 2; };
 template <> struct StaticShape<9> { static constexpr int KD = 7, KH = 7, KW = 1, LW = 2, LH = 3, LD = 3; };
 template <> struct StaticShape<16> { static constexpr int KD = 1, KH = 3, KW = 3, LW = 4, LH = 4, LD = 0; };
 template <> struct StaticShape<12> { static constexpr int KD = 3, KH = 2, KW = 2, LW = 2, LH = 2, LD = 4; };
@@ -62,7 +66,7 @@
     return 1;
 #else
     if (CK == 64 && WCH == 4 && WPX == 8 && ST == 1) return 2;
-    if (CK == 32 && WCH == 5 && WPX == 8 && (ST == 7 || ST == 8 || ST == 9)) return 2;
+    if (CK == 32 && WCH == 5 && WPX == 8 && halo_t256(ST)) return 2;
     if (CK == 64 && WCH == 2 && WPX == 8 && WVP == 2 && ST == 16) return 2;
     if (CK == 32 && WCH == 2 && WPX == 8 && ST == 1 && MODE == MODE_SPADE) return 2;
 #ifdef CS_LDS_V32
@@ -73,8 +77,8 @@
 }
 template <int ST, int PAD> constexpr int halo_hi()
 {
-    if (PAD == 2) return ST == 3 ? 16 : (ST == 9 ? 19 : ((ST == 7 || ST == 8) ? 15 : (ST == 16 ? 13 : 8)));
-    return ST == 4 ? 18 : ((ST == 3 || ST == 7 || ST == 8 || ST == 9) ? 13 : (ST == 12 ? 9 : 8));
+    if (PAD == 2) return ST == 3 ? 16 : (ST == 9 ? 19 : ((ST == 7 || ST == 8 || ST == 18) ? 15 : (ST == 16 ? 13 : 8)));
+    return ST == 4 ? 18 : ((ST == 3 || halo_t256(ST)) ? 13 : (ST == 12 ? 9 : 8));
 }
 template <int ST, int PAD> __host__ __device__ constexpr int halo_lane_pos(int l)
 {
@@ -112,6 +116,24 @@
     for (int u = g + 1; u <= NP; ++u) carried += WCH + (u < NP ? dma(u, true) : 0);
     carried += cur_before(0);
     return prime < carried ? prime : carried;
+}
+
+template <int ST, int PAD, int MODE, int BM, int WCH, int EP_WPX, int EPCODE>
+__device__ __forceinline__ void halo_ep_frags(const ConvParams& p, f4_t (&ep_acc)[WCH][EP_WPX], int ep_wpx, int ep_prot, int wch, int n0,
+                                              int tw, int th, int td, int tn, int tile_lin, int lane)
+{
+    using SS = StaticShape<ST>;
+    constexpr int lgTW = SS::LW, lgTH = SS::LH, lgTD = SS::LD, lgS = lgTW + lgTH + lgTD;
+    constexpr int mW = (1 << lgTW) - 1, mH = (1 << lgTH) - 1, mD = (1 << lgTD) - 1;
+    constexpr int EP_PAIR = 0, EP_POOL_WSH_K = 0, EP_POOL_HSH_K = 0;
+    constexpr bool EP_EARLY = false, EP_HEAVY = false;
+    const unsigned ep_o0_extra = 0u;
+    const ep_u2_t ep_xpre[1][1] = {};
+    const int l15 = lane & 15, l4 = lane >> 4, l15p = halo_lane_pos<ST, PAD>(l15);
+#ifdef CS_TIMELINE
+    unsigned long long tl_t[8];
+#endif
+    CONV_EPILOGUE_IMPL(EPCODE);
 }
 
 template <int ST, int PAD> constexpr int halo_pool_shift(int bit)
@@ -181,9 +203,14 @@
     const int phz = (PHK && p.nphase) ? (int)blockIdx.z : 0;
     const int PHv = (PHK && p.nphase) ? p.ph_PH[phz] : p.PH, PWv = (PHK && p.nphase) ? p.ph_PW[phz] : p.PW;
     const unsigned ep_o0_extra = (PHK && p.nphase) ? p.ph_ooff[phz] : 0u;
+    constexpr int ep_prot = 0;
+    constexpr bool T144 = halo_t144(ST);
+    static_assert(!T144 || (DB && !SK && CK == 32 && WCH == 5 && WPX == 8 && WVP == 2 && MODE == MODE_STD), "the nine-fragment form is a form of the 256 x 160 ASMR kernel");
+    constexpr int ACH = T144 ? 4 : WCH;
     const int wpx = SK ? 0 : wave % WVP, wch = SK ? 0 : wave / WVP;
     const int l15 = lane & 15, l4 = lane >> 4;
     const int l15p = halo_lane_pos<ST, PAD>(l15);
+    const int prot = T144 ? wch * (WPX / 2) : 0;
 #ifdef CS_NO_PAIR
     constexpr int EP_PAIR = 0;
 #else
@@ -192,8 +219,9 @@
 
 #ifdef CS_NO_ASMRING
     constexpr bool ASMRK = false;
-#else
-    constexpr bool ASMRK = DB && !SK && CK == 32 && WCH == 5 && WPX == 8 && WVP == 2 && (ST == 7 || ST == 8 || ST == 9) && MODE == MODE_STD;
+    static_assert(!halo_t144(ST), "the nine-fragment form is a form of the 256 x 160 ASMR kernel");
+#else
+    constexpr bool ASMRK = DB && !SK && CK == 32 && WCH == 5 && WPX == 8 && WVP == 2 && halo_t256(ST) && MODE == MODE_STD;
 #endif
     u4_t wr_p[ASMRK ? 3 : 1][ASMRK ? WCH : 1];
     unsigned poffb[ASMRK ? HI : 1];
@@ -307,7 +335,7 @@
     int abase[WPX];
 #pragma unroll
     for (int pi = 0; pi < WPX; ++pi) {
-        int m = wpx * WPX * 16 + pi * 16 + l15p;
+        int m = wpx * WPX * 16 + (pi ^ prot) * 16 + l15p;
         const int wl = m & mW; m >>= lgTW;
         const int hl = m & mH; m >>= lgTH;
         const int dl = m & mD; m >>= lgTD;
@@ -321,7 +349,8 @@
     const half_t* wbase = p.wgt;
     if (p.wslot) wbase += p.wofs[p.wslot[nb < p.N ? nb : p.N - 1]];
     if (PHK && p.nphase) wbase += p.ph_wofs[phz];
-    const half_t* wlane = wbase + ((long)(n0 + wch * WCH * 16) * 32 + ep_lane_row(EP_PAIR, l15) * 32 + l4 * 8);
+    const half_t* wlane = wbase + ((long)(n0 + wch * ACH * 16) * 32 + ep_lane_row(EP_PAIR, l15) * 32 + l4 * 8);
+    const int w4off = (T144 ? 8 - 4 * wch : 4) * 16 * 32;
     const long wstep = (long)p.Cout_pad * 32;
 
 #ifdef CS_NO_EARLY
@@ -338,15 +367,18 @@
     const int ep_wpx0 = wpx;
     CONV_EPILOGUE_EARLY_FETCH()
 
-    f4_t acc[WCH][WPX];
-#pragma unroll
-    for (int ci = 0; ci < WCH; ++ci)
+    f4_t acc[ACH][WPX];
+    f4_t acc9[1][T144 ? WPX / 2 : 1];
+#pragma unroll
+    for (int ci = 0; ci < ACH; ++ci)
 #pragma unroll
         for (int pi = 0; pi < WPX; ++pi) acc[ci][pi] = (f4_t){0.f, 0.f, 0.f, 0.f};
+#pragma unroll
+    for (int pi = 0; pi < (T144 ? WPX / 2 : 1); ++pi) acc9[0][pi] = (f4_t){0.f, 0.f, 0.f, 0.f};
 
     if constexpr (ST != 0) {
         constexpr int NT = SS::KD * SS::KH * SS::KW, NS = NT * KH32;
-        constexpr bool RAGK = (CK == 32) && (WPX == 8) && (ST == 7 || ST == 8 || ST == 9) && MODE == MODE_STD;
+        constexpr bool RAGK = (CK == 32) && (WPX == 8) && halo_t256(ST) && MODE == MODE_STD;
         constexpr bool LATK = CK == 64 && WCH == 2 && WPX == 4 && ST == 1 && !SK;
 #ifdef CS_PFS3
         constexpr int PFS = NS < 3 ? NS : 3;
@@ -366,7 +398,7 @@
 #ifdef CS_NO_ASMRING
         constexpr bool ASMR = false;
 #else
-        constexpr bool ASMR = DB && WCH == 5 && WPX == 8 && WVP == 2 && (ST == 7 || ST == 8 || ST == 9) && MODE == MODE_STD && PFS == 3;
+        constexpr bool ASMR = DB && WCH == 5 && WPX == 8 && WVP == 2 && halo_t256(ST) && MODE == MODE_STD && PFS == 3;
 #endif
         if constexpr (ASMR) {
             static_assert(SK == false && KH32 == 1, "ASMR: 32-channel chunks");
@@ -409,7 +441,7 @@
                 else if (ci == 1) asm volatile("global_load_dwordx4 %0, %1, off offset:1024" : "=v"(dst) : "v"(src));
                 else if (ci == 2) asm volatile("global_load_dwordx4 %0, %1, off offset:2048" : "=v"(dst) : "v"(src));
                 else if (ci == 3) asm volatile("global_load_dwordx4 %0, %1, off offset:3072" : "=v"(dst) : "v"(src));
-                else asm volatile("global_load_dwordx4 %0, %1, off" : "=v"(dst) : "v"(src + 4 * 16 * 32));
+                else asm volatile("global_load_dwordx4 %0, %1, off" : "=v"(dst) : "v"(src + w4off));
             };
             static_assert(EP_PAIR == 0, "ASMR: plain weight row order");
             TL_STAMP(1);
@@ -479,19 +511,22 @@
 #pragma unroll
                     for (int k = 0; k < 2 * WCH; ++k) {
                         const int ci = k >> 1, p0 = (k & 1) * 2;
-                        acc[ci][p0] = __builtin_amdgcn_mfma_f32_16x16x32_f16(__builtin_bit_cast(h8_t, wr[st % PFS][ci]), afA[p0], acc[ci][p0], 0, 0, 0);
-                        acc[ci][p0 + 1] = __builtin_amdgcn_mfma_f32_16x16x32_f16(__builtin_bit_cast(h8_t, wr[st % PFS][ci]), afA[p0 + 1], acc[ci][p0 + 1], 0, 0, 0);
+                        f4_t& a0 = (T144 && ci >= ACH) ? acc9[0][T144 ? p0 : 0] : acc[ci < ACH ? ci : 0][p0];
+                        f4_t& a1 = (T144 && ci >= ACH) ? acc9[0][T144 ? p0 + 1 : 0] : acc[ci < ACH ? ci : 0][p0 + 1];
+                        a0 = __builtin_amdgcn_mfma_f32_16x16x32_f16(__builtin_bit_cast(h8_t, wr[st % PFS][ci]), afA[p0], a0, 0, 0, 0);
+                        a1 = __builtin_amdgcn_mfma_f32_16x16x32_f16(__builtin_bit_cast(h8_t, wr[st % PFS][ci]), afA[p0 + 1], a1, 0, 0, 0);
                         if (k >= 2 && k < 6) afB[k - 2] = *(const h8_t*)(hb + ab_of(HA + k - 2, st) + toff);
                         if constexpr (st >= 1) { if (k >= 5) wload1(wr[(st - 1) % PFS][k - 5], rsrc_w, k - 5); }
                         __builtin_amdgcn_sched_barrier(0);
                     }
                     if (st >= ST0 && st < ST0 + HI) { stage_piece(nbuf, cc + 1, st - ST0); __builtin_amdgcn_sched_barrier(0); }
-#pragma unroll
-                    for (int k = 0; k < 2 * WCH; ++k) {
+                    constexpr int RD0 = T144 ? 1 : 2;
+#pragma unroll
+                    for (int k = 0; k < 2 * ACH; ++k) {
                         const int ci = k >> 1, p0 = (k & 1) * 2;
                         acc[ci][HA + p0] = __builtin_amdgcn_mfma_f32_16x16x32_f16(__builtin_bit_cast(h8_t, wr[st % PFS][ci]), afB[p0], acc[ci][HA + p0], 0, 0, 0);
                         acc[ci][HA + p0 + 1] = __builtin_amdgcn_mfma_f32_16x16x32_f16(__builtin_bit_cast(h8_t, wr[st % PFS][ci]), afB[p0 + 1], acc[ci][HA + p0 + 1], 0, 0, 0);
-                        if (k >= 2 && k < 6 && st + 1 < NSC) afA[k - 2] = *(const h8_t*)(hb + ab_of(k - 2, st + 1) + toff_of(st + 1));
+                        if (k >= RD0 && k < RD0 + 4 && st + 1 < NSC) afA[k - RD0] = *(const h8_t*)(hb + ab_of(k - RD0, st + 1) + toff_of(st + 1));
                         __builtin_amdgcn_sched_barrier(0);
                     }
                 });
@@ -721,7 +756,16 @@
     constexpr bool EP_HEAVY = (MODE == MODE_PIXSHUF) || (WCH == 1) || (ST == 15) || (ST == 0);
     constexpr bool KWSUM = !SK && MODE == MODE_STD && WCH == 5 && WPX == 8 && WVP == 2 && (ST == 8 || ST == 9);
     TL_STAMP(3);
-    if constexpr (!SK) {
+    if constexpr (T144) {
+        constexpr int E0 = EP_CODE(0, 1, 0, 0, 0);
+        if (!p.ep_general && p.Cout == 144 && !p.out0_f32) {
+            halo_ep_frags<ST, PAD, MODE, BM, ACH, WPX, E0>(p, acc, wpx, prot, wch, n0, tw, th, td, tn, tile_lin, lane);
+            halo_ep_frags<ST, PAD, MODE, BM, 1, WPX / 2, E0>(p, acc9, wpx * 2 + wch, 0, 8, n0, tw, th, td, tn, tile_lin, lane);
+        } else {
+            halo_ep_frags<ST, PAD, MODE, BM, ACH, WPX, -1>(p, acc, wpx, prot, wch, n0, tw, th, td, tn, tile_lin, lane);
+            halo_ep_frags<ST, PAD, MODE, BM, 1, WPX / 2, -1>(p, acc9, wpx * 2 + wch, 0, 8, n0, tw, th, td, tn, tile_lin, lane);
+        }
+    } else if constexpr (!SK) {
         if (p.sk_out) {
             const long mtot = (long)p.N * p.D * p.H * p.W;
 #pragma unroll
@@ -969,6 +1013,17 @@
     constexpr int BM = SK ? WPX * 16 : WPX * 16 * WVP, BN = WCH * 16 * WVC;
     constexpr int PAD = halo_pad<CK, WPX, WCH, WVP, ST, MODE>(), HI = halo_hi<ST, PAD>();
     constexpr int SLP = CK / 8 + PAD, VS = SLP * 16;
+    constexpr bool T144 = halo_t144(ST);
+    if constexpr (T144) {
+        if (p.Cout_pad != 160 || p.Cout <= 128 || p.Cout > 144 || p.Cout % 4) {
+            cs_set_error("conv_halo: the 256 x 144 tile computes rows 0 - 143 of 160 packed ones: 128 < Cout <= 144, a multiple of 4 (Cout %d, Cout_pad %d)", p.Cout, p.Cout_pad);
+            return -1;
+        }
+        const char* why = p.res.p ? "a residual" : p.out1.p ? "a second output" : p.stat_out ? "statistics" : p.pool_hw ? "pooling" : (p.sk_out || p.sk_splits) ? "split-K" :
+                          p.kw_out ? "the kw sum (kw_out)" : p.pixscale ? "a per-position scale" : (p.spmul || p.xs_w) ? "the spmul forms" : p.nphase ? "a grouped launch" :
+                          !p.out0.p ? "no out0" : nullptr;
+        if (why) { cs_set_error("conv_halo: the 256 x 144 tile's epilogue is bias + activation into one out0; this launch asks for %s", why); return -1; }
+    }
     if (p.Cout_pad % BN != 0) { cs_set_error("conv_halo: Cout_pad %d not a multiple of the channel tile %d", p.Cout_pad, BN); return -1; }
     {
         const long in_span = (long)(p.N - 1) * p.in_sN + (long)(p.D - 1) * p.in_sD + (long)(p.H - 1) * p.in_sH + (long)(p.W - 1) * p.in_sW +
@@ -1027,7 +1082,7 @@
     if (MODE == MODE_SPADE && (1 << lgS) != BM) { cs_set_error("conv_halo: SPADE launches must tile within one sample"); return -1; }
     if (MODE == MODE_SPADE && p.res_f32) { cs_set_error("conv_halo: the tensor a SPADE launch modulates is fp16"); return -1; }
     if (p.ragged) {
-        constexpr bool ragk = (CK == 32) && (WPX == 8) && (ST == 7 || ST == 8 || ST == 9) && MODE == MODE_STD;
+        constexpr bool ragk = (CK == 32) && (WPX == 8) && halo_t256(ST) && MODE == MODE_STD;
         if (!ragk || SK || p.Cin % 32 != 16 || p.sk_out || p.hilo || p.cg > 0) {
             cs_set_error("conv_halo: paired-tap weights (ragged) need the 256-position 32-channel static kernels and Cin %% 32 == 16");
             return -1;
@@ -1043,7 +1098,7 @@
     const int nck = (p.Cin + CK - 1) / CK;
     constexpr bool big = (BM == 256 && WCH == 5);
 #ifndef CS_NO_ASMRING
-    constexpr bool asmr = WCH == 5 && WPX == 8 && WVP == 2 && (ST == 7 || ST == 8 || ST == 9) && MODE == MODE_STD && !SK;
+    constexpr bool asmr = WCH == 5 && WPX == 8 && WVP == 2 && halo_t256(ST) && MODE == MODE_STD && !SK;
 #else
     constexpr bool asmr = false;
 #endif
@@ -1099,15 +1154,19 @@
         kp.persist_total = (int)total;
         grid = dim3(total < 256u ? (total + 7u) & ~7u : 256u, 1);
     }
+    if constexpr (T144) {
+        if (!(asmr && db)) { cs_set_error("conv_halo: the 256 x 144 tile exists as the double-buffered ASMR kernel only (two or more channel chunks)"); return -1; }
+    }
+    constexpr int ST_DB = (T144 && !asmr) ? 7 : ST, ST_SB = T144 ? 7 : ST;
     if (db) {
-        auto k = conv_halo_kernel<CK, WPX, WCH, WVP, WVC, MODE, true, SK, ST>;
+        auto k = conv_halo_kernel<CK, WPX, WCH, WVP, WVC, MODE, true, SK, ST_DB>;
         if (lds > 64 * 1024) {
             e = hipFuncSetAttribute((const void*)k, hipFuncAttributeMaxDynamicSharedMemorySize, (int)lds);
             if (e != hipSuccess) { cs_set_error("conv_halo: opting into %zu bytes of LDS failed: %s", lds, hipGetErrorString(e)); return -1; }
         }
         hipLaunchKernelGGL(k, grid, dim3(256), lds, st, kp);
     } else {
-        auto k = conv_halo_kernel<CK, WPX, WCH, WVP, WVC, MODE, false, SK, ST>;
+        auto k = conv_halo_kernel<CK, WPX, WCH, WVP, WVC, MODE, false, SK, ST_SB>;
         if (lds > 64 * 1024) {
             e = hipFuncSetAttribute((const void*)k, hipFuncAttributeMaxDynamicSharedMemorySize, (int)lds);
             if (e != hipSuccess) { cs_set_error("conv_halo: opting into %zu bytes of LDS failed: %s", lds, hipGetErrorString(e)); return -1; }
diff --git a/canonswap_amd/csrc/engine.hip b/canonswap_amd/csrc/engine.hip
--- a/canonswap_amd/csrc/engine.hip
+++ b/canonswap_amd/csrc/engine.hip
@@ -240,6 +240,7 @@
 
 int cfg_v32() { return CFG_H_256x32; }
 
+bool tail144() { static const bool on = [] { const char* s = getenv("CANONSWAP_TAIL144"); return !s || atoi(s) != 0; }(); return on; }
 constexpr int HALO_PERSIST = 1;
 constexpr int XCD_MAP = 2;
 
@@ -285,7 +286,8 @@
             const int NT = c.p.KD * c.p.KH * c.p.KW, PK = c.p.KW > 1 ? c.p.KW : c.p.KH;
             ksteps -= NT - (NT / PK) * (PK / 2 + PK % 2);
         }
-        e->flops_exec += 2.0 * (double)c.p.N * c.p.D * c.p.H * c.p.W * c.p.Cout_pad * 32.0 * ksteps * nph;
+        const int rows = c.hcfg == CFG_H_256x144 ? 144 : c.p.Cout_pad;
+        e->flops_exec += 2.0 * (double)c.p.N * c.p.D * c.p.H * c.p.W * rows * 32.0 * ksteps * nph;
     }
     if (vol32_enabled() && vol32_supported(c.p) && (c.p.N >= VOL32_MINB || c.p.stat_out || c.p.xf_kind)) {
         if (e->latency_mode && c.p.stat_out) c.p.v32_srows = 2;
@@ -310,7 +312,7 @@
     }
     if (c.p.inD == c.p.D) {
         const int hcfg = c.hcfg >= 0 ? c.hcfg : pick_halo_cfg(c.p, c.mode);
-        const int BM = (hcfg == CFG_H_256x32 || hcfg == CFG_H_256x16 || hcfg == CFG_H_256x160 || hcfg == CFG_H_256x64) ? 256 : 128;
+        const int BM = (hcfg == CFG_H_256x32 || hcfg == CFG_H_256x16 || hcfg == CFG_H_256x160 || hcfg == CFG_H_256x144 || hcfg == CFG_H_256x64) ? 256 : 128;
         const bool is3d = c.p.KD > 1;
         if (!prefW) { prefW = is3d ? 8 : 16; prefH = is3d ? 8 : BM / 16; }
         set_tile(c.p, BM, prefW, prefH);
@@ -328,12 +330,12 @@
         {
             const bool sk_on = e->latency_mode;
             const int bn = hcfg == CFG_H_128x256 ? 256 : hcfg == CFG_H_128x128 ? 128 : hcfg == CFG_H_128x64 || hcfg == CFG_H_256x64 ? 64 :
-                           hcfg == CFG_H_128x160 || hcfg == CFG_H_256x160 ? 160 : hcfg == CFG_H_128x16 || hcfg == CFG_H_256x16 ? 16 : 32;
+                           hcfg == CFG_H_128x160 || hcfg == CFG_H_256x160 || hcfg == CFG_H_256x144 ? 160 : hcfg == CFG_H_128x16 || hcfg == CFG_H_256x16 ? 16 : 32;
             const long wgs = (long)c.p.nTW * c.p.nTH * c.p.nTD * c.p.nTN * (c.p.Cout_pad / bn);
             const int nck = (c.p.Cin + ck - 1) / ck;
             const long mtot = (long)c.p.N * c.p.D * c.p.H * c.p.W;
             const bool plain = c.mode == MODE_STD && !c.p.res.p && !c.p.pixscale && !c.p.out1.p && !c.p.stat_out && !c.p.s2 &&
-                               c.p.act0 <= ACT_SIGMOID && c.p.out0.p && hcfg != CFG_H_SK128x32 && c.p.Cout % 4 == 0 && !c.p.spmul && !c.p.nphase &&
+                               c.p.act0 <= ACT_SIGMOID && c.p.out0.p && hcfg != CFG_H_SK128x32 && hcfg != CFG_H_256x144 && c.p.Cout % 4 == 0 && !c.p.spmul && !c.p.nphase &&
                                (!c.p.pool_hw || (!c.p.out0_f32 && !(c.p.H & 1) && !(c.p.W & 1)));
             constexpr int sk_maxwg = 64, sk_fill = 512;
             if (sk_on && plain && wgs <= sk_maxwg && nck >= 4 && e->sk_buf) {
@@ -531,7 +533,7 @@
     }
     ConvCall t = mk(e->w_tail, e->dm_l[0], dhwc(nullptr, FD, 64, 64, 144), B, FD, 64, 64);
     t.p.act0 = ACT_RELU; t.p.out0 = dhwc(e->dm_pred, FD, 64, 64, 144);
-    t.hcfg = CFG_H_256x160;
+    t.hcfg = tail144() ? CFG_H_256x144 : CFG_H_256x160;
     TRY(go(e, t, st));
     ConvCall m = mk(e->w_mask, e->dm_pred, dhwc(nullptr, FD, 64, 64, 144), B, FD, 64, 64);
     m.p.kw_out = e->dm_logits;
@@ -1624,7 +1626,7 @@
     if (d->cfg == CFG_LAT) return launch_conv_lat(p, c.mode, (hipStream_t)stream);
     if (d->cfg >= 10 || d->cfg == -2) {
         const int hcfg = d->cfg >= 10 ? d->cfg : pick_halo_cfg(p, c.mode);
-        const int BM = (hcfg == CFG_H_256x32 || hcfg == CFG_H_256x16 || hcfg == CFG_H_256x160 || hcfg == CFG_H_256x64) ? 256 : 128;
+        const int BM = (hcfg == CFG_H_256x32 || hcfg == CFG_H_256x16 || hcfg == CFG_H_256x160 || hcfg == CFG_H_256x144 || hcfg == CFG_H_256x64) ? 256 : 128;
         const bool is3d = p.KD > 1;
         set_tile(p, BM, d->tile_w ? d->tile_w : (is3d ? 8 : 16), d->tile_h ? d->tile_h : (is3d ? 8 : BM / 16));
         const int ck = d->ck ? d->ck : ((!is3d && p.Cin % 64 == 0) ? 64 : 32);
```

After: 547.7 frames/s, median of 6. Within noise of the previous version (+0.4%).
